# moddyz/stereo-to-multiview-cuda

Measured on AMD Instinct MI355X. Metric: stereo->8-view frames/sec @1080p d=64; cost-agg HBM GB/s vs roofline, higher is better.
Workload: dtype f32; 1 GPU; 1920x1080 synthetic stereo frame, D=64, zd=32, full stereo->8-view frame: cost init + cross aggregation + WTA + DCC/IRV x5/bilateral + 6 DIBR views + interlacing, one frame per GPU per step; stages=3, usd=34, lsd=17, views=8, aggregation=matrix pipe (stm_kernels_aggm.hip)

## Files before the change

include/stm_hip.h:

```cpp
#ifndef STM_HIP_H
#define STM_HIP_H

#ifdef __cplusplus
extern "C" {
#endif
#if defined(STM_BUILD) && defined(__GNUC__)
#pragma GCC visibility push(default)
#endif

int         stm_version(void);
void        stm_set_stream(void *hip_stream);
void       *stm_get_stream(void);
void        stm_set_error_mode(int mode);
const char *stm_last_error(void);
void        stm_release_workspace(void);
void        stm_prof_enable(int on);
void        stm_prof_reset(void);
int         stm_prof_read(const char *kernel, float *total_ms);
void        stm_set_agg_variant(int v);
int         stm_agg_path(int num_disp, int zero_disp, int num_rows, int num_cols, int usd, int stages);
int         stm_first_pass_path(int num_disp, int zero_disp, int num_rows, int num_cols, int usd, int stages);
void        stm_set_irv_paper_ratio(int on);
int         stm_set_irv_chunk(int entries);
int         stm_irv_path(int num_rows, int num_cols, int usd, int iterations, int device_flavour, int with_dcc);
int         stm_set_lens(int mode, double pitch, double slope, double centre);
int         stm_set_depth(int mode, float gain, float conv);
int         stm_set_depth_auto(float disp_lo, float disp_hi, float max_gain, int clip_permille, float rate, float *d_state);
int         stm_set_antialias(int mode, float strength, int max_radius, float gate);
void        stm_get_antialias(int out_mode[2], float out[2]);
int         stm_set_align(int mode, float a, float b, float c);
int         stm_set_align_auto(int radius, float rate, float *d_state);
void        stm_get_align(int out_mode[2], float out[4]);
int         stm_set_balance(int mode, const unsigned char *lut768);
int         stm_set_balance_auto(int max_shift, float rate, int *d_state);
void        stm_get_balance(int out_mode[2], float *out_rate, unsigned char out_lut[768]);
int         stm_set_cut(int mode, int thresh_permille, int min_gap, int *d_state);
void        stm_get_cut(int out[3]);
int         stm_set_layout(int layout, int tiles_x, int tiles_y, int order, int filter);
void        stm_get_layout(int *out);
int         stm_set_output(int format, int matrix, int pitch, int uv_row);
void        stm_get_output(int out[4]);
int         stm_set_overlay(int mode, const unsigned char *d_overlay, int ov_rows, int ov_cols, int x0, int y0, float disparity);
void        stm_get_overlay(int out[5], float *disparity);
void        stm_set_quilt_lds_limit(int bytes);
int         stm_set_packing(int packing, int swap, int filter, int gap);
void        stm_get_packing(int *out);
void        stm_set_ref_quirks(int on);

void stm_ci_adcensus(unsigned char *img_l, unsigned char *img_r, float **cost_l, float **cost_r,
                     float ad_coeff, float census_coeff, int num_disp, int zero_disp,
                     int num_rows, int num_cols, int elem_sz);
void stm_d_ci_adcensus(unsigned char *d_img_l, unsigned char *d_img_r,
                       float **d_adcensus_cost_l, float **d_adcensus_cost_r,
                       float **h_adcensus_cost_l, float **h_adcensus_cost_r,
                       float *d_adcensus_cost_memory,
                       float ad_coeff, float census_coeff, int num_disp, int zero_disp,
                       int num_rows, int num_cols, int elem_sz);

void stm_ca_cross(unsigned char *img, unsigned char **cross, float **cost, float **acost,
                  float ucd, float lcd, int usd, int lsd,
                  int num_disp, int num_rows, int num_cols, int elem_sz);
void stm_d_ca_cross(unsigned char *d_img, float **d_cost,
                    float **d_acost, float **h_acost, float *d_acost_memory,
                    unsigned char **d_cross,
                    float ucd, float lcd, int usd, int lsd,
                    int num_disp, int num_rows, int num_cols, int elem_sz);

void stm_dc_wta(float **cost, float *disp, int num_disp, int zero_disp, int num_rows, int num_cols);
void stm_d_dc_wta(float **d_cost, float *d_disp, int num_disp, int zero_disp, int num_rows, int num_cols);
void stm_dc_subpixel(float **cost, float *disp, int num_disp, int zero_disp, int num_rows, int num_cols);
void stm_d_dc_subpixel(float **d_cost, float *d_disp, int num_disp, int zero_disp, int num_rows, int num_cols);
void stm_dc_hslo(float **cost, float *disp, unsigned char *img_l, unsigned char *img_r,
                 float T, float H1, float H2, int num_disp, int zero_disp,
                 int num_rows, int num_cols, int elem_sz);
void stm_d_dc_hslo(float **d_cost, float *d_disp, unsigned char *d_img_l, unsigned char *d_img_r,
                   float T, float H1, float H2, int num_disp, int zero_disp,
                   int num_rows, int num_cols, int elem_sz);

void stm_dr_dcc(unsigned char *outliers_l, unsigned char *outliers_r, float *disp_l, float *disp_r,
                int num_rows, int num_cols);
void stm_d_dr_dcc(unsigned char *d_outliers_l, unsigned char *d_outliers_r, float *d_disp_l, float *d_disp_r,
                  int num_rows, int num_cols);
void stm_dr_irv(float *disp, unsigned char *outliers, unsigned char **cross, int thresh_s, float thresh_h,
                int num_rows, int num_cols, int num_disp, int zero_disp, int usd, int iterations);
void stm_d_dr_irv(float *d_disp, unsigned char *d_outliers, unsigned char **d_cross, int thresh_s, float thresh_h,
                  int num_rows, int num_cols, int num_disp, int zero_disp, int usd, int iterations);
void stm_dr_interp(float *disp, unsigned char *outliers, unsigned char *img, int num_rows, int num_cols, int elem_sz);
void stm_d_dr_interp(float *d_disp, unsigned char *d_outliers, unsigned char *d_img, int num_rows, int num_cols, int elem_sz);
void stm_filter_bilateral_1(float *img, int radius, float sigma_color, float sigma_spatial,
                            int num_rows, int num_cols, int num_disp);
void stm_d_filter_bilateral_1(float *d_img, int radius, float sigma_color, float sigma_spatial,
                              int num_rows, int num_cols, int num_disp);
void stm_filter_gaussian_1(float *img, int radius, float sigma_spatial, int num_rows, int num_cols);
void stm_d_filter_gaussian_1(float *d_img, int radius, float sigma_spatial, int num_rows, int num_cols);
void stm_filter_bleed_1(unsigned char *img, int radius, int num_rows, int num_cols);
void stm_d_filter_bleed_1(unsigned char *d_img, int radius, int num_rows, int num_cols);
void stm_filter_median(float *img, int num_rows, int num_cols);
void stm_d_filter_median(float *d_img, int num_rows, int num_cols);

void stm_dibr_occl(unsigned char *occl_l, unsigned char *occl_r, float *disp_l, float *disp_r,
                   int num_rows, int num_cols);
void stm_d_dibr_occl(unsigned char *d_occl_l, unsigned char *d_occl_r, float *d_disp_l, float *d_disp_r,
                     int num_rows, int num_cols);
void stm_dibr_occl_to_mask(float *mask_l, float *mask_r, unsigned char *occl_l, unsigned char *occl_r,
// ... 228 lines not shown
```

stereo-to-multiview-cuda_amd/_lib.py:

```python
import ctypes as C
import os

HERE = os.path.dirname(os.path.abspath(__file__))
LIB_PATH = os.path.join(HERE, "libstm_hip.so")
if os.environ.get("STM_LIB") == "timing":
    LIB_PATH = os.path.join(HERE, "libstm_hip_timing.so")

u8p = C.POINTER(C.c_uint8)
f32p = C.POINTER(C.c_float)
u32p = C.POINTER(C.c_uint32)
u8pp = C.POINTER(u8p)
f32pp = C.POINTER(f32p)
vp = C.c_void_p
i, f, d = C.c_int, C.c_float, C.c_double

PROTOS = {
    "stm_version": ([], i),
    "stm_set_stream": ([vp], None),
    "stm_get_stream": ([], vp),
    "stm_set_error_mode": ([i], None),
    "stm_last_error": ([], C.c_char_p),
    "stm_release_workspace": ([], None),
    "stm_prof_enable": ([i], None),
    "stm_prof_reset": ([], None),
    "stm_prof_read": ([C.c_char_p, f32p], i),
    "stm_set_agg_variant": ([i], None),
    "stm_agg_path": ([i, i, i, i, i, i], i),
    "stm_first_pass_path": ([i, i, i, i, i, i], i),
    "stm_set_irv_paper_ratio": ([i], None),
    "stm_set_irv_chunk": ([i], i),
    "stm_irv_path": ([i, i, i, i, i, i], i),
    "stm_set_ref_quirks": ([i], None),
    "stm_set_lens": ([i, d, d, d], i),
    "stm_set_layout": ([i, i, i, i, i], i),
    "stm_get_layout": ([C.POINTER(C.c_int)], None),
    "stm_set_output": ([i, i, i, i], i),
    "stm_get_output": ([C.POINTER(C.c_int)], None),
    "stm_set_overlay": ([i, vp, i, i, i, i, f], i),
    "stm_get_overlay": ([C.POINTER(C.c_int), f32p], None),
    "stm_set_quilt_lds_limit": ([i], None),
    "stm_set_packing": ([i, i, i, i], i),
    "stm_get_packing": ([C.POINTER(C.c_int)], None),
    "stm_set_depth": ([i, f, f], i),
    "stm_set_depth_auto": ([f, f, f, i, f, vp], i),
    "stm_set_antialias": ([i, f, i, f], i),
    "stm_get_antialias": ([C.POINTER(C.c_int), f32p], None),
    "stm_set_align": ([i, f, f, f], i),
    "stm_set_align_auto": ([i, f, vp], i),
    "stm_get_align": ([C.POINTER(C.c_int), f32p], None),
    "stm_set_balance": ([i, u8p], i),
    "stm_set_balance_auto": ([i, f, vp], i),
    "stm_get_balance": ([C.POINTER(C.c_int), f32p, u8p], None),
    "stm_set_cut": ([i, i, i, vp], i),
    "stm_get_cut": ([C.POINTER(C.c_int)], None),
    "stm_ci_adcensus": ([u8p, u8p, f32pp, f32pp, f, f, i, i, i, i, i], None),
    "stm_d_ci_adcensus": ([vp, vp, vp, vp, f32pp, f32pp, vp, f, f, i, i, i, i, i], None),
    "stm_ca_cross": ([u8p, u8pp, f32pp, f32pp, f, f, i, i, i, i, i, i], None),
    "stm_d_ca_cross": ([vp, vp, vp, f32pp, vp, vp, f, f, i, i, i, i, i, i], None),
    "stm_dc_wta": ([f32pp, f32p, i, i, i, i], None),
    "stm_d_dc_wta": ([vp, vp, i, i, i, i], None),
    "stm_dc_subpixel": ([f32pp, f32p, i, i, i, i], None),
    "stm_d_dc_subpixel": ([vp, vp, i, i, i, i], None),
    "stm_dc_hslo": ([f32pp, f32p, u8p, u8p, f, f, f, i, i, i, i, i], None),
    "stm_d_dc_hslo": ([vp, vp, vp, vp, f, f, f, i, i, i, i, i], None),
    "stm_dr_dcc": ([u8p, u8p, f32p, f32p, i, i], None),
    "stm_d_dr_dcc": ([vp, vp, vp, vp, i, i], None),
    "stm_dr_irv": ([f32p, u8p, u8pp, i, f, i, i, i, i, i, i], None),
    "stm_d_dr_irv": ([vp, vp, vp, i, f, i, i, i, i, i, i], None),
    "stm_dr_interp": ([f32p, u8p, u8p, i, i, i], None),
    "stm_d_dr_interp": ([vp, vp, vp, i, i, i], None),
    "stm_filter_bilateral_1": ([f32p, i, f, f, i, i, i], None),
    "stm_d_filter_bilateral_1": ([vp, i, f, f, i, i, i], None),
    "stm_filter_gaussian_1": ([f32p, i, f, i, i], None),
    "stm_d_filter_gaussian_1": ([vp, i, f, i, i], None),
    "stm_filter_bleed_1": ([u8p, i, i, i], None),
    "stm_d_filter_bleed_1": ([vp, i, i, i], None),
    "stm_filter_median": ([f32p, i, i], None),
    "stm_generate_gaussian_kernel": ([f32p, i, f], None),
    "stm_d_filter_median": ([vp, i, i], None),
    "stm_dibr_occl": ([u8p, u8p, f32p, f32p, i, i], None),
    "stm_d_dibr_occl": ([vp, vp, vp, vp, i, i], None),
    "stm_dibr_occl_to_mask": ([f32p, f32p, u8p, u8p, i, i], None),
    "stm_d_dibr_occl_to_mask": ([vp, vp, vp, vp, i, i], None),
    "stm_dibr_dbm": ([u8p, u8p, u8p, f32p, f32p, u8p, u8p, f32p, f32p, f, i, i, i], None),
    "stm_d_dibr_dbm": ([vp, vp, vp, vp, vp, vp, vp, vp, vp, f, i, i, i], None),
    "stm_dibr_dbm_lin": ([u8p, u8p, u8p, f32p, f32p, u8p, u8p, f32p, f32p, f, i, i, i], None),
    "stm_d_dibr_dbm_lin": ([vp, vp, vp, vp, vp, vp, vp, vp, vp, f, i, i, i], None),
    "stm_dibr_dfm": ([u8p, u8p, u8p, f32p, f32p, f, i, i, i], None),
    "stm_d_dibr_dfm": ([vp, vp, vp, vp, vp, f, i, i, i], None),
    "stm_mux_multiview": ([u8pp, u8p, i, f, i, i, i, i, i], None),
    "stm_d_mux_multiview": ([vp, vp, i, f, i, i, i, i, i], None),
    "stm_mux_multiview_lens": ([u8pp, u8p, i, i, d, d, d, i, i, i, i, i], None),
    "stm_d_mux_multiview_lens": ([vp, vp, i, i, d, d, d, i, i, i, i, i], None),
    "stm_quilt_multiview": ([u8pp, u8p, i, i, i, i, i, i, i, i, i, i], None),
    "stm_d_quilt_multiview": ([vp, vp, i, i, i, i, i, i, i, i, i, i], None),
    "stm_mux_overlay": ([u8p, u8p, i, i, i, i, f, i, f, i, d, d, d, i, i, i, i, i, i, i], None),
    "stm_d_mux_overlay": ([vp, vp, i, i, i, i, f, i, f, i, d, d, d, i, i, i, i, i, i, i], None),
    "stm_d_demux_sbs": ([vp, vp, vp, i, i, i, i], None),
    "stm_demux_nv12": ([u8p, u8p, u8p, i, u8p, i, i, i, i, i, i], None),
    "stm_d_demux_nv12": ([vp, vp, vp, i, vp, i, i, i, i, i, i], None),
    "stm_mux_nv12": ([u8p, i, u8p, i, u8p, i, i, i, i], None),
    "stm_d_mux_nv12": ([vp, i, vp, i, vp, i, i, i, i], None),
    "stm_demux_packed": ([u8p, u8p, u8p, i, i, i, i, i, i, i, i], None),
    "stm_d_demux_packed": ([vp, vp, vp, i, i, i, i, i, i, i, i], None),
    "stm_demux_nv12_packed": ([u8p, u8p, u8p, i, u8p, i, i, i, i, i, i, i, i, i, i], None),
    "stm_d_demux_nv12_packed": ([vp, vp, vp, i, vp, i, i, i, i, i, i, i, i, i, i], None),
    "stm_adcensus_stm": ([u8p, f32p, f32p, u8p, i, i, i, i, i, i, i, f, i, i, f, f, f, f, i, i, i, f], None),
    "stm_d_adcensus_stm": ([vp, vp, vp, vp, i, i, i, i, i, i, i, f, i, i, f, f, f, f, i, i, i, f, i], None),
    "stm_d_adcensus_stm_t": ([vp, vp, vp, vp, i, i, i, i, i, i, i, f, i, i, f, f, f, f, i, i, i, f, i, vp, vp, vp, f, i, f], None),
    "stm_d_adcensus_stm_nv12": ([vp, i, vp, i, i, vp, vp, vp, i, i, i, i, i, i, i, f, i, i, f, f, f, f, i, i, i, f, i, vp, vp, vp, vp, f, i, f,
                                 vp, vp], None),
# ... 82 lines not shown
```

stereo-to-multiview-cuda_amd/csrc/stm_api.hip:

```cpp
#include "stm_common.h"
#include <initializer_list>
#include <mutex>
#include "../../include/stm_hip.h"

#include <map>
#include <stdio.h>
#include <stdlib.h>
#include <string.h>
#include <tuple>
#include <vector>

using namespace stm;

namespace {

struct DevTable {
    float *d = nullptr;
    size_t n = 0;
};
std::map<std::tuple<int, int, float, float>, DevTable> g_tables;

int cur_dev()
{
    int dev = 0;
// ... 51 lines not shown
const float *bilateral_one_value_table(int D, int zd, float sigma_spatial, float sigma_color)
{
    if (D < 1 || D >= (1 << 19) || zd < 0 || zd >= 4096) return nullptr;
    return dev_table(3, D * 4096 + zd, sigma_spatial, sigma_color, (size_t)D, fill_bil1);
}

void sync() { STM_CHECK(hipStreamSynchronize(stream())); }

template <class T> T *up(const T *h, size_t n)
{
    T *d = Workspace::get<T>(n);
    STM_CHECK(hipMemcpyAsync(d, h, n * sizeof(T), hipMemcpyHostToDevice, stream()));
    return d;
}
template <class T> void down(T *h, const T *d, size_t n)
{
    STM_CHECK(hipMemcpyAsync(h, d, n * sizeof(T), hipMemcpyDeviceToHost, stream()));
}
float *up_planes(float **planes, int D, size_t HW)
{
    float *slab = Workspace::get<float>((size_t)D * HW);
    for (int d = 0; d < D; ++d)
        STM_CHECK(hipMemcpyAsync(slab + (size_t)d * HW, planes[d], HW * sizeof(float), hipMemcpyHostToDevice, stream()));
    return slab;
}
void down_planes(float **planes, const float *slab, int D, size_t HW)
{
    for (int d = 0; d < D; ++d)
        STM_CHECK(hipMemcpyAsync(planes[d], slab + (size_t)d * HW, HW * sizeof(float), hipMemcpyDeviceToHost, stream()));
}

struct Arms {
    u8 *up, *down, *left, *right;
};

struct Dim { const char *name; int v, lo; };
bool args_ok(const char *fn, std::initializer_list<Dim> dims)
{
    if (api_outermost()) clear_failed();
    for (const Dim &d : dims)
        if (d.v < d.lo) {
            char msg[160];
            snprintf(msg, sizeof msg, "%s: %s = %d, must be >= %d", fn, d.name, d.v, d.lo);
            fail(msg, d.name, __FILE__, __LINE__);
            return false;
        }
    return true;
}


void core_ci(const u8 *d_img_l, const u8 *d_img_r, Vol cl, Vol cr, uint32_t *pk_l, uint32_t *pk_r, float ad_coeff,
             float census_coeff, int D, int zd, int H, int W, int elem_sz, bool packed_ready = false,
             uint32_t **census_out = nullptr, uint32_t *const *census_ready = nullptr)
{
    size_t HW = (size_t)H * W;
    uint32_t *cen_l = census_ready ? census_ready[0] : Workspace::get<uint32_t>(HW), *cen_r = census_ready ? census_ready[1] : Workspace::get<uint32_t>(HW);
    if (!packed_ready) {
        launch_pack_bgrx(d_img_l, pk_l, H, W, elem_sz);
        launch_pack_bgrx(d_img_r, pk_r, H, W, elem_sz);
    }
    if (!census_ready) launch_census32_pair(pk_l, cen_l, pk_r, cen_r, H, W);
    if (census_out) {
        census_out[0] = cen_l;
        census_out[1] = cen_r;
        return;
    }
    const float *lut = rho_table(ad_coeff, census_coeff);
    launch_cost_init(pk_l, pk_r, cen_l, cen_r, cl, cr, lut, lut + 768, D, zd, H, W);
    if (ref_quirks()) launch_cost_quirks(pk_l, pk_r, cen_l, cen_r, cl, cr, lut, lut + 768, D, zd, H, W);
}

static bool agg_on_matrix_pipe(int usd, int H, int W) { return (agg_variant() / 10000) % 10 != 1 && aggm_supports(usd, H, W); }
static bool stages_hslo(int stages) { return (stages & 0x100) != 0; }
static bool stages_subpix(int stages) { return (stages & 0x200) != 0; }
int frame_agg_path(int D, int zd, int H, int W, int usd, int stages)
{
    if (D < 1 || H < 1 || W < 1 || !agg_on_matrix_pipe(usd, H, W)) return 0;
    return 1 | aggm_frame_path(D, zd, H, W, usd, stages_hslo(stages), stages_subpix(stages));
}
int frame_first_pass_path(int D, int zd, int H, int W, int usd, int stages)
{
    if (D < 1 || H < 1 || W < 1 || !agg_on_matrix_pipe(usd, H, W)) return 0;
    return aggm_frame_hc2_parts(D, zd, H, W, usd, stages_hslo(stages), stages_subpix(stages));
}
void core_agg(Vol cost, Vol scratch, const Arms &a, int D, int H, int W, int usd)
{
    if (agg_on_matrix_pipe(usd, H, W) && launch_aggm_stage(cost, cost, a.up, a.down, a.left, a.right, D, H, W, usd)) return;
    if (!scratch.base && !scratch.tab) scratch = vol_slab(Workspace::get<float>((size_t)D * H * W), (size_t)H * W);
    launch_agg_h(cost, scratch, a.left, a.right, D, H, W);
    launch_agg_v(scratch, cost, a.up, a.down, D, H, W, usd);
    launch_agg_v(cost, scratch, a.up, a.down, D, H, W, usd);
    launch_agg_h(scratch, cost, a.left, a.right, D, H, W);
}
Arms carve_arms(size_t HW)
{
    u8 *m = Workspace::get<u8>(4 * HW);
    return Arms{m, m + HW, m + 2 * HW, m + 3 * HW};
}
Arms arms_from_table(unsigned char **d_cross)
{
    u8 *h[4];
    STM_CHECK(hipMemcpyAsync(h, d_cross, sizeof h, hipMemcpyDeviceToHost, stream()));
    sync();
    return Arms{h[0], h[1], h[2], h[3]};
}

void core_bilateral(float *d_img, int radius, float sigma_color, float sigma_spatial, int H, int W, int D)
{
    size_t HW = (size_t)H * W;
    float *tmp = Workspace::get<float>(HW);
    launch_bilateral(d_img, tmp, gauss2d_table(radius, sigma_spatial), gauss1d_table(D, sigma_color), radius, H, W, D);
    STM_CHECK(hipMemcpyAsync(d_img, tmp, HW * sizeof(float), hipMemcpyDeviceToDevice, stream()));
}

void core_dbm(u8 *d_out, const u8 *d_l, const u8 *d_r, const float *disp_l, const float *disp_r, const float *mask_l,
              const float *mask_r, float shift, int H, int W, int elem_sz, int g_radius, float g_sigma, bool linear = false)
{
    size_t HW = (size_t)H * W;
    float *blend = Workspace::get<float>(HW);
    launch_gaussian_max(mask_r, blend, gauss2d_table(g_radius, g_sigma), g_radius, g_sigma, H, W, true);
    launch_view_synth(d_out, d_l, d_r, disp_l, disp_r, mask_l, mask_r, blend, shift, H, W, elem_sz, linear);
}

void dbm_device(const char *fn, unsigned char *d_img_out, unsigned char *d_img_in_l, unsigned char *d_img_in_r, float *d_disp_l,
                float *d_disp_r, float *d_mask_l, float *d_mask_r, float shift, int num_rows, int num_cols, int elem_sz, bool linear)
{
    if (!args_ok(fn, {{"num_rows", num_rows, 1}, {"num_cols", num_cols, 1}, {"elem_sz", elem_sz, 3}})) return;
    Workspace::begin((size_t)num_rows * num_cols * 4 + 1024);
    if (elem_sz > 3)
        STM_CHECK(hipMemsetAsync(d_img_out, 0, (size_t)num_rows * num_cols * elem_sz, stream()));
    core_dbm(d_img_out, d_img_in_l, d_img_in_r, d_disp_l, d_disp_r, d_mask_l, d_mask_r, shift, num_rows, num_cols, elem_sz,
             10, 15.0f, linear);
}
void dbm_host(const char *fn, unsigned char *img_out, unsigned char *img_in_l, unsigned char *img_in_r, float *disp_l, float *disp_r,
              float *mask_l, float *mask_r, float shift, int num_rows, int num_cols, int elem_sz, bool linear)
{
    if (!args_ok(fn, {{"num_rows", num_rows, 1}, {"num_cols", num_cols, 1}, {"elem_sz", elem_sz, 3}})) return;
    size_t HW = (size_t)num_rows * num_cols;
    Workspace::begin(3 * HW * elem_sz + 20 * HW + 8192);
    u8 *l = up(img_in_l, HW * elem_sz), *r = up(img_in_r, HW * elem_sz), *o = Workspace::get<u8>(HW * elem_sz);
    float *dl = up(disp_l, HW), *dr = up(disp_r, HW), *ml = up(mask_l, HW), *mr = up(mask_r, HW);
    STM_CHECK(hipMemsetAsync(o, 0, HW * elem_sz, stream()));
    core_dbm(o, l, r, dl, dr, ml, mr, shift, num_rows, num_cols, elem_sz, 7, 10.0f, linear);
    down(img_out, o, HW * elem_sz);
    sync();
}

bool mux_geom_ok(int N, float angle, int elem_sz, float *y_interval, float *inv_y_interval, int *ymod_out)
{
    float yi = mux_y_interval(N, angle, elem_sz);
    if (!(fabsf(yi) < 1.0e9f)) {
        fail("mux_multiview: y_interval is not finite (tan(angle) == 0 or angle is not a number)", "angle", __FILE__, __LINE__);
        return false;
    }
    int ymod = (int)roundf(yi);
    if (ymod == 0) {
        fail("mux_multiview: round(y_interval) == 0 (angle too steep)", "ymod", __FILE__, __LINE__);
        return false;
    }
    if (y_interval) *y_interval = yi;
    if (inv_y_interval) *inv_y_interval = 1.0f / yi;
    if (ymod_out) *ymod_out = ymod;
    return true;
}
void core_mux(const u8 *const *d_views, u8 *d_out, int N, float angle, int Hin, int Win, int Hout, int Wout, int elem_sz,
              int variant)
// ... 1690 lines not shown
    } else if (pack_on) {
        launch_demux_packed(img_l, img_r, pin, H, W, elem_sz);
        fused_split = false;
    } else if (nv && (agg_variant() / 100) % 10 != 6) {
        for (int i = 0; i < 6; ++i) pre[i] = Workspace::get<uint32_t>(HW);
        launch_front_nv12(img_l, img_r, pre[0], pre[1], pre[2], pre[3], pre[4], pre[5], nv->y, nv->pitch_y, nv->uv, nv->pitch_uv, H, W,
                          elem_sz, nv->matrix);
    } else if (nv) {
        launch_demux_nv12(img_l, img_r, nv->y, nv->pitch_y, nv->uv, nv->pitch_uv, H, W, elem_sz, nv->matrix);
        fused_split = false;
    } else if (fused_split && (agg_variant() / 100) % 10 != 6) {
        for (int i = 0; i < 6; ++i) pre[i] = Workspace::get<uint32_t>(HW);
        launch_front(img_l, img_r, pre[0], pre[1], pre[2], pre[3], pre[4], pre[5], d_img_sbs, H, num_cols_sbs, W, elem_sz);
    } else if (fused_split) {
        for (int i = 0; i < 4; ++i) pre[i] = Workspace::get<uint32_t>(HW);
        launch_demux_sbs_packed(img_l, img_r, pre[0], pre[1], pre[2], pre[3], d_img_sbs, H, num_cols_sbs, W, elem_sz);
    } else {
        launch_demux_sbs(img_l, img_r, d_img_sbs, H, num_cols_sbs, W, elem_sz);
    }
    Arms al, ar;
    const bool hslo = stages_hslo(stages), subpix = stages_subpix(stages);
    const bool interp = (stages & 0x400) != 0;
    const bool linwarp = (stages & 0x800) != 0;
    stages &= 0xff;
    frame_disparity(img_l, img_r, d_disp_l, d_disp_r, al, ar, H, W, elem_sz, num_disp, zero_disp, ad_coeff, census_coeff, ucd,
                    lcd, usd, lsd, thresh_s, thresh_h, stages >= 2, hslo, fused_split ? pre : nullptr, subpix, interp);
    if (hist) {
        float *c[2] = {d_disp_l, d_disp_r};
        const float *q[2] = {hist->disp_l, hist->disp_r};
        const bool split = split_hist || pack_on;
        const u8 *prev_l = hist->img_l, *prev_r = hist->img_r;
        if (pack_on && !nv) {
            u8 *ul = Workspace::get<u8>(IMG), *ur = Workspace::get<u8>(IMG);
            PackInput prev = pin;
            prev.frame = hist->sbs;
            launch_demux_packed(ul, ur, prev, H, W, elem_sz);
            prev_l = ul;
            prev_r = ur;
        }
        const u8 *im[2] = {split ? img_l : d_img_sbs, split ? img_r : d_img_sbs}, *ip[2] = {split ? prev_l : hist->sbs, split ? prev_r : hist->sbs};
        const size_t off[2] = {0, split ? 0 : (size_t)W * elem_sz};
        launch_disp_temporal(2, c, q, im, ip, off, H, W, split ? W : num_cols_sbs, elem_sz, hist->alpha, hist->thresh_color, hist->thresh_disp);
    }
    if (stages < 3) return;
    frame_render(img_l, img_r, d_disp_l, d_disp_r, d_interlaced, H, W, num_rows_out, num_cols_out, elem_sz, N, angle, linwarp);
    if (overlay().mode == 1) frame_overlay(d_interlaced, overlay(), lens(), layout(), N, angle, num_rows_out, num_cols_out, elem_sz);
}

bool frame_dims_ok(const char *fn, int num_rows, int num_cols_sbs, int num_cols, int num_rows_out, int num_cols_out, int elem_sz,
                   int num_views, int num_disp)
{
    return args_ok(fn, {{"num_rows", num_rows, 1}, {"num_cols_sbs", num_cols_sbs, 1}, {"num_cols", num_cols, 1},
                        {"num_rows_out", num_rows_out, 1}, {"num_cols_out", num_cols_out, 1}, {"elem_sz", elem_sz, 3},
                        {"num_views", num_views, 2}, {"num_disp", num_disp, 1}});
}

bool frame_packing_ok(const char *fn, int num_rows, int num_cols_sbs, int num_cols)
{
    const Packing pk = packing();
    return !pk.on() || packing_args_ok(fn, pk, num_rows, num_cols_sbs, num_cols, "num_cols", false, 0, 0, 0);
}
bool packing_unsupported(const char *fn)
{
    if (!packing().on()) return false;
    char msg[200];
    snprintf(msg, sizeof msg, "%s: a packing is set on this thread (stm_set_packing), which this call does not support: use d_adcensus_stm, "
             "d_adcensus_stm_t or d_adcensus_stm_nv12", fn);
    fail(msg, "packing", __FILE__, __LINE__);
    return true;
}

}

extern "C" {

int stm_agg_path(int num_disp, int zero_disp, int num_rows, int num_cols, int usd, int stages)
{
    return frame_agg_path(num_disp, zero_disp, num_rows, num_cols, usd, stages);
}
int stm_first_pass_path(int num_disp, int zero_disp, int num_rows, int num_cols, int usd, int stages)
{
    return frame_first_pass_path(num_disp, zero_disp, num_rows, num_cols, usd, stages);
}

void stm_d_adcensus_stm(unsigned char *d_img_sbs, float *d_disp_l, float *d_disp_r, unsigned char *d_interlaced,
                        int num_rows, int num_cols_sbs, int num_cols, int num_rows_out, int num_cols_out, int elem_sz,
                        int num_views, float angle, int num_disp, int zero_disp, float ad_coeff, float census_coeff,
                        float ucd, float lcd, int usd, int lsd, int thresh_s, float thresh_h, int stages)
{
    if (!frame_dims_ok("d_adcensus_stm", num_rows, num_cols_sbs, num_cols, num_rows_out, num_cols_out, elem_sz, num_views, num_disp)) return;
    if (!frame_packing_ok("d_adcensus_stm", num_rows, num_cols_sbs, num_cols)) return;
    if (stages & 0x2000) {
        fail("d_adcensus_stm: stages 0x2000 (temporal stabilisation) needs the history arguments of d_adcensus_stm_t", "stages", __FILE__,
             __LINE__);
        return;
    }
    frame_device("d_adcensus_stm", d_img_sbs, d_disp_l, d_disp_r, d_interlaced, num_rows, num_cols_sbs, num_cols, num_rows_out, num_cols_out,
                 elem_sz, num_views, angle, num_disp, zero_disp, ad_coeff, census_coeff, ucd, lcd, usd, lsd, thresh_s, thresh_h, stages, nullptr);
}

void stm_d_adcensus_stm_t(unsigned char *d_img_sbs, float *d_disp_l, float *d_disp_r, unsigned char *d_interlaced,
                          int num_rows, int num_cols_sbs, int num_cols, int num_rows_out, int num_cols_out, int elem_sz,
                          int num_views, float angle, int num_disp, int zero_disp, float ad_coeff, float census_coeff,
                          float ucd, float lcd, int usd, int lsd, int thresh_s, float thresh_h, int stages,
                          unsigned char *d_prev_img_sbs, float *d_prev_disp_l, float *d_prev_disp_r, float alpha, int thresh_color,
                          float thresh_disp)
{
    const char *fn = "d_adcensus_stm_t";
    if (!frame_dims_ok(fn, num_rows, num_cols_sbs, num_cols, num_rows_out, num_cols_out, elem_sz, num_views, num_disp)) return;
    if (!frame_packing_ok(fn, num_rows, num_cols_sbs, num_cols)) return;
    TemporalHist hist = {d_prev_img_sbs, d_prev_disp_l, d_prev_disp_r, alpha, thresh_color, thresh_disp};
    bool run = false;
    if (stages & 0x2000) {
        const int nset = (d_prev_img_sbs != nullptr) + (d_prev_disp_l != nullptr) + (d_prev_disp_r != nullptr);
        const size_t HW = (size_t)num_rows * num_cols;
        if (!temporal_params_ok(fn, alpha, thresh_color, thresh_disp)) return;
        if ((stages & 0xff) < 2) {
            fail("d_adcensus_stm_t: stages 0x2000 (temporal stabilisation) needs the refinement stages (2 or 3)", "stages", __FILE__, __LINE__);
            return;
        }
        if (nset != 0 && nset != 3) {
            fail("d_adcensus_stm_t: the three history pointers must be all null (first frame) or all set", "d_prev_img_sbs, d_prev_disp_l, d_prev_disp_r",
                 __FILE__, __LINE__);
            return;
        }
        if (nset == 3 && !packing().on() && num_cols_sbs < 2 * num_cols) {
            fail("d_adcensus_stm_t: stages 0x2000 (temporal stabilisation) needs num_cols_sbs >= 2 * num_cols", "num_cols_sbs", __FILE__, __LINE__);
            return;
        }
        if (nset == 3 && (maps_overlap(d_prev_disp_l, d_disp_l, HW) || maps_overlap(d_prev_disp_l, d_disp_r, HW) ||
                          maps_overlap(d_prev_disp_r, d_disp_l, HW) || maps_overlap(d_prev_disp_r, d_disp_r, HW))) {
            fail("d_adcensus_stm_t: a history map must not alias d_disp_l or d_disp_r", "d_prev_disp_l, d_prev_disp_r", __FILE__, __LINE__);
            return;
        }
        run = nset == 3;
    }
    frame_device(fn, d_img_sbs, d_disp_l, d_disp_r, d_interlaced, num_rows, num_cols_sbs, num_cols, num_rows_out, num_cols_out, elem_sz,
                 num_views, angle, num_disp, zero_disp, ad_coeff, census_coeff, ucd, lcd, usd, lsd, thresh_s, thresh_h, stages & ~0x2000,
                 run ? &hist : nullptr);
}

void stm_d_adcensus_stm_nv12(unsigned char *d_y, int pitch_y, unsigned char *d_uv, int pitch_uv, int matrix, float *d_disp_l, float *d_disp_r,
                             unsigned char *d_interlaced, int num_rows, int num_cols_sbs, int num_cols, int num_rows_out, int num_cols_out,
                             int elem_sz, int num_views, float angle, int num_disp, int zero_disp, float ad_coeff, float census_coeff,
                             float ucd, float lcd, int usd, int lsd, int thresh_s, float thresh_h, int stages,
                             unsigned char *d_prev_img_l, unsigned char *d_prev_img_r, float *d_prev_disp_l, float *d_prev_disp_r, float alpha,
                             int thresh_color, float thresh_disp, unsigned char *d_img_l, unsigned char *d_img_r)
{
    const char *fn = "d_adcensus_stm_nv12";
    if (!frame_dims_ok(fn, num_rows, num_cols_sbs, num_cols, num_rows_out, num_cols_out, elem_sz, num_views, num_disp)) return;
    if (packing().on()) {
        if (!packing_args_ok(fn, packing(), num_rows, num_cols_sbs, num_cols, "num_cols", true, pitch_y, pitch_uv, matrix)) return;
    } else if (!nv12_args_ok(fn, num_rows, num_cols_sbs, num_cols, "num_cols", pitch_y, pitch_uv, matrix)) return;
    if ((d_img_l != nullptr) != (d_img_r != nullptr)) {
        fail("d_adcensus_stm_nv12: d_img_l and d_img_r must be both null (the split images stay in the workspace) or both set", "d_img_l, d_img_r",
             __FILE__, __LINE__);
        return;
    }
    TemporalHist hist = {nullptr, d_prev_disp_l, d_prev_disp_r, alpha, thresh_color, thresh_disp, d_prev_img_l, d_prev_img_r};
    Nv12Input nv = {d_y, d_uv, pitch_y, pitch_uv, matrix, d_img_l, d_img_r};
    bool run = false;
    if (stages & 0x2000) {
        const int nset = (d_prev_img_l != nullptr) + (d_prev_img_r != nullptr) + (d_prev_disp_l != nullptr) + (d_prev_disp_r != nullptr);
        const size_t HW = (size_t)num_rows * num_cols, IMG = HW * elem_sz;
        if (!temporal_params_ok(fn, alpha, thresh_color, thresh_disp)) return;
        if ((stages & 0xff) < 2) {
// ... 505 lines not shown
```

stereo-to-multiview-cuda_amd/csrc/stm_common.h:

```cpp
#pragma once
#include <hip/hip_runtime.h>
#include <stddef.h>
#include <stdint.h>

typedef unsigned char u8;

namespace stm {

void fail(const char *what, const char *expr, const char *file, int line);
bool failed();
void clear_failed();
struct ApiNest { ApiNest(); ~ApiNest(); };
bool api_outermost();
void release_host_frame_bufs();
bool nv12_args_ok(const char *fn, int num_rows, int num_cols_sbs, int num_cols, const char *cols_name, int pitch_y, int pitch_uv, int matrix);
#define STM_CHECK(expr)                                                                  \
    do {                                                                                 \
        hipError_t _e = (expr);                                                          \
        if (_e != hipSuccess) ::stm::fail(hipGetErrorString(_e), #expr, __FILE__, __LINE__); \
    } while (0)
#define STM_CHECK_LAUNCH() STM_CHECK(hipGetLastError())
#define STM_LAUNCH(...)                                     \
    do {                                                    \
        if (!::stm::failed()) hipLaunchKernelGGL(__VA_ARGS__); \
// ... 244 lines not shown
void set_overlay(const Overlay &o);
bool overlay_params_ok(const char *fn, const void *ov, bool check_ptr, int ov_rows, int ov_cols, int x0, int y0, float disparity);
void frame_overlay(u8 *d_frame, const Overlay &ov, const Lens &ln, const Layout &lo, int num_views, float angle, int Hout, int Wout,
                   int elem_sz);
void launch_overlay(u8 *out, const u8 *ov, int ov_rows, int ov_cols, int x0, int y0, float disparity, int N, const Lens &ln,
                    float y_interval, float inv_y_interval, int ymod, const Layout &lo, int Hout, int Wout, int elem_sz);
struct Antialias {
    int mode;
    float strength;
    int max_radius;
    float gate;
};
Antialias antialias();
void set_antialias(const Antialias &a);
bool antialias_params_ok(const char *fn, float strength, int max_radius, float gate);
void launch_view_prefilter(int nimg, u8 *const *out, const u8 *const *in, const float *const *disp, int H, int W, int elem_sz, int num_views,
                           float strength, int max_radius, float gate, float gain, float conv, const float *state);
void launch_depth_fit(float *state, uint32_t *hist, const float *disp_l, const float *disp_r, int H, int W, float disp_lo, float disp_hi,
                      float max_gain, int clip_permille, float rate, bool fresh);
struct Align {
    int mode;
    float a, b, c;
    int radius;
    float rate;
    float *d_state;
};
Align align();
void set_align(const Align &a);
bool align_params_ok(const char *fn, int mode, float a, float b, float c);
bool align_auto_params_ok(const char *fn, int radius, float rate);
bool align_size_ok(const char *fn, int num_rows, int num_cols);
size_t align_profile_words(int H);
size_t align_sad_words(int radius);
void launch_align_measure(float *state, int *nvalid, uint32_t *prof, uint32_t *sad, const PackInput *in, const u8 *img_l, const u8 *img_r,
                          int H, int W, int elem_sz, int radius, float rate, bool fresh);
void launch_align_frame(u8 *out, const PackInput *in, const u8 *img, int H, int W, int elem_sz, float a, float b, float c, const float *state);
struct Balance {
    int mode;
    u8 lut[768];
    int max_shift;
    float rate;
    int *d_state;
};
Balance balance_default();
Balance balance();
void set_balance(const Balance &b);
bool balance_params_ok(const char *fn, int mode, const u8 *lut768);
bool balance_auto_params_ok(const char *fn, int max_shift, float rate);
bool balance_size_ok(const char *fn, int num_rows, int num_cols);
int balance_rate_q(float rate);
constexpr size_t BALANCE_HIST_WORDS = 1536, BALANCE_STATE_WORDS = 769;
void launch_balance_measure(int *state, uint32_t *hist, const PackInput *in, const u8 *img_l, const u8 *img_r, int H, int W, int elem_sz,
                            int max_shift, int rate_q, bool fresh);
void launch_balance_frame(u8 *out, const PackInput *in, const u8 *img, int H, int W, int elem_sz, const u8 *lut768, const int *state);
struct Cut {
    int mode;
    int thresh_permille, min_gap;
    int *d_state;
};
Cut cut_default();
Cut cut();
void set_cut(const Cut &c);
bool cut_params_ok(const char *fn, int thresh_permille, int min_gap);
bool cut_size_ok(const char *fn, int num_rows, int num_cols);
constexpr size_t CUT_SIG_WORDS = 256, CUT_STATE_WORDS = 260;
constexpr int CUT_DEFAULT_THRESH = 370;
void launch_cut_detect(int *state, uint32_t *sig, const PackInput *in, const u8 *img_l, int H, int W, int elem_sz, int thresh_permille,
                       int min_gap, void *reset0, void *reset1, void *reset2);
struct PQViews {
    const uint32_t *pk[2], *cen[2];
    float *a[2], *b[2];
    const u8 *armU[2], *armD[2], *armL[2], *armR[2];
    float *disp[2];
};
size_t pq_volume_floats(int D, int H, int W);
bool aggm_supports(int usd, int H, int W);
void launch_aggm_frame(const uint32_t *const *pk, const uint32_t *const *cen, const float *lut, float *const *vol_a, float *const *vol_b,
                       const u8 *const *armU, const u8 *const *armD, const u8 *const *armL, const u8 *const *armR, float *const *disp,
                       int D, int zd, int H, int W, int usd, bool keep_volume = false, uint32_t *htab_ready = nullptr, uint32_t *vtab_ready = nullptr,
                       bool v2_read_later = false);
size_t aggm_frame_htab_dwords(int D, int H, int W, int usd, bool keep_volume);
size_t aggm_frame_vtab_dwords(int D, int zd, int H, int W, int usd, bool keep_volume, bool v2_read_later, int *rec, int *top, bool *col);
bool aggm_frame_px(int D, int zd, int H, int W, int usd, bool keep_volume, bool v2_read_later);
int aggm_frame_path(int D, int zd, int H, int W, int usd, bool keep_volume, bool v2_read_later);
int aggm_frame_hc2_parts(int D, int zd, int H, int W, int usd, bool keep_volume, bool v2_read_later);
bool launch_aggm_stage(Vol in, Vol out, const u8 *armU, const u8 *armD, const u8 *armL, const u8 *armR, int D, int H, int W, int usd);
size_t aggm_stage_bytes(int D, int H, int W, int usd);
bool aggh_supports(int usd, int D);
size_t aggh_table_dwords(int nviews, int H, int W);
void launch_hwin_table(PQViews &v, int nviews, uint32_t *tab, int H, int W);
void launch_pq_hsr(PQViews &v, int nviews, const uint32_t *tab, int D, int zd, int H, int W, bool px = false);
bool aggv_supports(int usd);
int aggv_table_top();
int aggv_table_rec();
void launch_pq_v12q(PQViews &v, int nviews, const uint32_t *tab, int rec, int H, int W, int G, int NC);
void launch_pq_v12r(PQViews &v, int nviews, const uint32_t *tab, int H, int W, int G);
void launch_vcol_table(PQViews &v, int nviews, uint32_t *tab, int H, int W);
size_t aggv_col_table_dwords(int nviews, int H, int W);
void launch_to_pq(Vol in, float *pq, int D, int H, int W, uint32_t *odd = nullptr);
void launch_from_pq(const float *pq, Vol out, int D, int H, int W);
void launch_hslo_wta(int nviews, const Vol *cost, const u8 *const *img_a, const u8 *const *img_b, const int *osign,
                     float *const *disp, float T, float H1, float H2, int D, int zd, int H, int W, int elem_sz);
void launch_hslo_wta_pq(int nviews, float *const *cost_pq, float *const *acc_pq, const u8 *const *img_a, const u8 *const *img_b,
                        const int *osign, float *const *disp, float T, float H1, float H2, int D, int zd, int H, int W, int elem_sz);

void rho_luts(float ad_coeff, float census_coeff, float *lut_ad , float *lut_census );
void gaussian_kernel_2d(float *kernel, int radius, float sigma);
void gaussian_kernel_1d(float *kernel, int size, float sigma);
float mux_y_interval(int num_views, float angle, int elem_sz);

}
```

stereo-to-multiview-cuda_amd/csrc/stm_kernels_aggh.hip:

```cpp
#include "stm_hwin.h"
#include <cstdlib>

namespace stm {

__global__ __launch_bounds__(256) void stm_k_hwin_table(PQViews v, uint32_t *__restrict__ tab, int H, int W, int nTx)
{
    __shared__ uint32_t ev_all[4][4 * 96];
    const int wv = threadIdx.x >> 6, y = blockIdx.y, view = blockIdx.z;
    const int x0 = (blockIdx.x * 4 + wv) * 64, x = x0 + (threadIdx.x & 63);
    const u8 *__restrict__ armL = view ? v.armL[1] : v.armL[0], *__restrict__ armR = view ? v.armR[1] : v.armR[0];
    int aL = 0, aR = 0;
    if (x < W) {
        aL = armL[(size_t)y * W + x];
        aR = armR[(size_t)y * W + x];
    }
    hwin_build(tab + (size_t)view * H * nTx * HR_REC, ev_all[wv], y, x0, aL, aR, W, nTx);
}

template <int EXP, bool PX>
__global__ __launch_bounds__(64, 3) void stm_k_pq_hsr(PQViews pv, const uint32_t *__restrict__ htab, int D, int zd, int H, int W, int G, int NC, int nTx,
                                                      int parts, int nviews)
{
    const int part = blockIdx.x % parts, rest = blockIdx.x / parts, y = rest % H, view = rest / H;
    if (view >= nviews) return;
    const int per = (nTx + parts - 1) / parts, t0 = part * per, t1 = min(nTx, t0 + per);
    if (t0 >= t1) return;
    const int l = threadIdx.x;
    const float *in = view ? pv.a[1] : pv.a[0];
    float *disp_row = (view ? pv.disp[1] : pv.disp[0]) + (size_t)y * W;
    const uint32_t *hrec = htab + ((size_t)(view * H + y) * nTx + t0) * HR_REC;
    const uint32_t cstride = (uint32_t)H * (uint32_t)G * 256u;
    const uint32_t nrec = (uint32_t)NC * cstride;
    const int vload = PX ? 4 * l : (l >> 4) * (int)cstride + (l & 15) * 16;
    const int vn = l & 15;
    const int vst = (l & 15) == 0 ? (l >> 4) * 16 : 0x7ffffff0;
    float vbig[4];
#pragma unroll
    for (int b = 0; b < 4; ++b) vbig[b] = (16 * b + (l & 15)) >= D ? 3.402823466e+38f : 0.0f;
    const int yG = y * G, Gm1 = G - 1, W4 = W * 4;
    const float zdf = (float)zd;
    asm volatile(R"ASM(
        .set HR_EXP, %[exp]
        .set HR_PX, %[px]
        ; ---------------------------------------------------------------- macros
        ; one block of a sweep: four MFMAs on one pixel group (its four registers = four window steps), the A operand (lanes 16 a + m =
        ; step a, pixel m) shared through CBSZ / ABID.  p = block index, acur / anxt = the A registers of this / the next block
        .macro HR_BLOCK p, acur, anxt
        s_set_gpr_idx_idx s30
        v_mfma_f32_16x16x1_4b_f32 v[120:135], v[\acur], v0, v[120:135] cbsz:2 abid:0
        v_cndmask_b32_e64 v[\anxt], 0, 1.0, s[36+2*((\p)+1):37+2*((\p)+1)]
        v_mfma_f32_16x16x1_4b_f32 v[120:135], v[\acur], v1, v[120:135] cbsz:2 abid:1
        s_add_u32 s30, s30, 4
        s_cmp_eq_u32 s30, s29
        s_cselect_b32 s30, 0, s30
        v_mfma_f32_16x16x1_4b_f32 v[120:135], v[\acur], v2, v[120:135] cbsz:2 abid:2
        v_mfma_f32_16x16x1_4b_f32 v[120:135], v[\acur], v3, v[120:135] cbsz:2 abid:3
        .endm
        .macro HR_PAIR b
        HR_BLOCK 2*(\b), 136, 137
        HR_BLOCK 2*(\b)+1, 137, 136
        .endm
        ; in: s84 = q0 (first group of the sweep inside the range), s85 = n (1 .. 22), s26 = ring index of the range start.
        ; out: s90 = entry block 22 - n, s30 = ring index of the sweep's first group
        .macro HR_SWEEP_ISSUE
        s_sub_u32 s90, 22, s85
        s_lshl_b32 s31, s84, 2
        s_add_u32 s30, s26, s31
        s_sub_u32 s31, s30, s29
        s_cmp_ge_u32 s30, s29
        s_cselect_b32 s30, s31, s30
        .endm
        ; the header and the 24 mask pairs (block p reads pair p + 1 for its successor, the entry block's own comes through M0) of
        ; tile s31 (index relative to t0) start travelling
        .macro HR_NEXT_MASKS
        s_lshl_b32 s31, s31, 8
        s_add_u32 s88, %[hrec_lo], s31
        s_addc_u32 s89, %[hrec_hi], 0
        s_load_dwordx2 s[86:87], s[88:89], 0x0
        .if (HR_EXP & 8) == 0
        s_load_dwordx16 s[36:51], s[88:89], 0x20
        s_load_dwordx16 s[52:67], s[88:89], 0x60
        s_load_dwordx16 s[68:83], s[88:89], 0xa0
        .endif
        .endm
        .macro HR_SWEEP_RUN
        s_lshl_b32 m0, s90, 1
        s_nop 0
        s_movrels_b64 s[94:95], s[36:37]      ; the entry block's mask
        v_cndmask_b32_e64 v136, 0, 1.0, s[94:95]
        v_cndmask_b32_e64 v137, 0, 1.0, s[94:95]
        s_set_gpr_idx_on s30, 0x2
        s_mul_i32 s31, s90, 56
        s_getpc_b64 s[92:93]
HR_pc_%=_\@:
        s_add_u32 s31, s31, HR_blk0_%=_\@-HR_pc_%=_\@+12
        s_add_u32 s92, s92, s31
        s_addc_u32 s93, s93, 0
        v_mfma_f32_16x16x1_4b_f32 v[120:135], v136, v0, 0 cbsz:2 abid:0
        s_setpc_b64 s[92:93]
HR_blk0_%=_\@:
        HR_PAIR 0
        HR_PAIR 1
        HR_PAIR 2
        HR_PAIR 3
        HR_PAIR 4
        HR_PAIR 5
        HR_PAIR 6
        HR_PAIR 7
        HR_PAIR 8
        HR_PAIR 9
        HR_PAIR 10
HR_end_%=_\@:
        .if (HR_end_%=_\@-HR_blk0_%=_\@) != 22*56
        .error "sweep blocks are not 56 bytes each"
        .endif
        s_set_gpr_idx_off
        s_nop 15
        s_nop 3
        .endm
        .macro HR_ZERO_ACC
        v_mov_b32 v120, 0
// ... 78 lines not shown
        v_min_i32_dpp v[\d2], v[\d2], v[\d2] row_ror:4 row_mask:0xf bank_mask:0xf
        v_min_i32_dpp v[\d3], v[\d3], v[\d3] row_ror:4 row_mask:0xf bank_mask:0xf
        v_min_i32_dpp v[\d0], v[\d0], v[\d0] row_ror:2 row_mask:0xf bank_mask:0xf
        v_min_i32_dpp v[\d1], v[\d1], v[\d1] row_ror:2 row_mask:0xf bank_mask:0xf
        v_min_i32_dpp v[\d2], v[\d2], v[\d2] row_ror:2 row_mask:0xf bank_mask:0xf
        v_min_i32_dpp v[\d3], v[\d3], v[\d3] row_ror:2 row_mask:0xf bank_mask:0xf
        v_min_i32_dpp v[\d0], v[\d0], v[\d0] row_ror:1 row_mask:0xf bank_mask:0xf
        v_min_i32_dpp v[\d1], v[\d1], v[\d1] row_ror:1 row_mask:0xf bank_mask:0xf
        v_min_i32_dpp v[\d2], v[\d2], v[\d2] row_ror:1 row_mask:0xf bank_mask:0xf
        v_min_i32_dpp v[\d3], v[\d3], v[\d3] row_ror:1 row_mask:0xf bank_mask:0xf
        .endm

        ; one step of the walk: tile s24; lb = the landing registers this step empties and refills
        .macro HR_STEP lb
        ; the groups loaded two steps ago (4 t + 9 .. 4 t + 12) -> ring (the first tile's came with the prologue)
        s_cmp_eq_u32 s24, %[t0]
        s_cbranch_scc1 HR_nomove_%=_\@
        .if (HR_EXP & 2) == 0
        .if HR_PX
        s_waitcnt vmcnt(24)                   ; issued since: 4 stores, 16 loads, 4 stores
        .else
        s_waitcnt vmcnt(12)                   ; issued since: 4 stores, 4 loads, 4 stores
        .endif
        .endif
        s_add_u32 s96, s26, 72                ; group 4 t + 9 = range start + 18 groups
        s_sub_u32 s31, s96, s29
        s_cmp_ge_u32 s96, s29
        s_cselect_b32 s96, s31, s96
        s_set_gpr_idx_on s96, 0x8
        HR_PUT4 \lb
        HR_PUT4 \lb+4
        HR_PUT4 \lb+8
        HR_PUT4 \lb+12
        s_set_gpr_idx_off
HR_nomove_%=_\@:
        ; groups 4 t + 17 .. 4 t + 20 (the new groups of tile t + 2) -> the landing registers just emptied
        s_lshl_b32 s97, s24, 2
        s_add_i32 s97, s97, 17
        HR_LOAD_GROUP \lb, 0
        HR_LOAD_GROUP \lb, 1
        HR_LOAD_GROUP \lb, 2
        HR_LOAD_GROUP \lb, 3
        ; ------------------------------------------------------------ the sweep of tile t (header and masks left after the last sweep)
        s_waitcnt lgkmcnt(0)
        s_mov_b32 s84, s86
        s_min_u32 s85, s87, 22
        s_cmp_eq_u32 s85, 0
        s_cbranch_scc1 HR_zero_%=_\@
        .if (HR_EXP & 1) == 0
        HR_SWEEP_ISSUE
        HR_SWEEP_RUN
        s_branch HR_wta_%=_\@
        .endif
HR_zero_%=_\@:
        HR_ZERO_ACC
HR_wta_%=_\@:
        ; the next tile's header and masks travel during WTA and the next ring update (the last tile reads its own again)
        s_add_i32 s31, s24, 1
        s_sub_u32 s91, %[t1], 1
        s_min_i32 s31, s31, s91
        s_sub_i32 s31, s31, %[t0]
        HR_NEXT_MASKS
        .if (HR_EXP & 4) == 0
        ; ------------------------------------------------------------ WTA (d_dc_wta.cu:19-34)
        s_cmp_eq_u32 s27, 0
        s_cbranch_scc1 HR_nofix_%=_\@
        v_max_f32 v120, v120, %[vb0]
        v_max_f32 v121, v121, %[vb0]
        v_max_f32 v122, v122, %[vb0]
        v_max_f32 v123, v123, %[vb0]
        v_max_f32 v124, v124, %[vb1]
        v_max_f32 v125, v125, %[vb1]
        v_max_f32 v126, v126, %[vb1]
        v_max_f32 v127, v127, %[vb1]
        v_max_f32 v128, v128, %[vb2]
        v_max_f32 v129, v129, %[vb2]
        v_max_f32 v130, v130, %[vb2]
        v_max_f32 v131, v131, %[vb2]
        v_max_f32 v132, v132, %[vb3]
        v_max_f32 v133, v133, %[vb3]
        v_max_f32 v134, v134, %[vb3]
        v_max_f32 v135, v135, %[vb3]
HR_nofix_%=_\@:
        ; per lane: the lowest of its four chunks, the lower chunk on ties; v[138:141] = that hypothesis (d = 16 b + n)
        HR_WTA_CHUNK 1, 151
        HR_WTA_CHUNK 2, 152
        HR_WTA_CHUNK 3, 153
        ; over the 16 hypothesis lanes: lowest cost (bit patterns: costs are never negative), then the lowest d among its holders
        HR_ROWMIN4 142, 143, 144, 145, 120, 121, 122, 123
        v_cmp_eq_u32_e64 s[94:95], v142, v120
        v_cmp_eq_u32_e64 s[96:97], v143, v121
        v_cmp_eq_u32_e64 s[98:99], v144, v122
        v_cmp_eq_u32_e64 s[90:91], v145, v123
        v_cndmask_b32_e64 v146, v150, v138, s[94:95]
        v_cndmask_b32_e64 v147, v150, v139, s[96:97]
        v_cndmask_b32_e64 v148, v150, v140, s[98:99]
        v_cndmask_b32_e64 v149, v150, v141, s[90:91]
        HR_ROWMIN4 142, 143, 144, 145, 146, 147, 148, 149
        v_cvt_f32_i32 v142, v142
        v_cvt_f32_i32 v143, v143
        v_cvt_f32_i32 v144, v144
        v_cvt_f32_i32 v145, v145
        v_subrev_f32 v142, %[zdf], v142
        v_subrev_f32 v143, %[zdf], v143
        v_subrev_f32 v144, %[zdf], v144
        v_subrev_f32 v145, %[zdf], v145
        .endif
        ; lane n == 0 of a pixel quad stores pixels 16 t + 4 q + i; pixels past the row are out of range (the whole offset is in
        ; the vector register, so the range check sees it).  Always four stores: a step's loads are counted against them
        s_lshl_b32 s31, s24, 6
        v_add_u32 v146, s31, %[vst]
        s_nop 0
        buffer_store_dword v142, v146, s[20:23], 0 offen
        buffer_store_dword v143, v146, s[20:23], 0 offen offset:4
        buffer_store_dword v144, v146, s[20:23], 0 offen offset:8
        buffer_store_dword v145, v146, s[20:23], 0 offen offset:12
        ; next tile
        s_add_u32 s26, s26, 16
        s_sub_u32 s31, s26, s29
        s_cmp_ge_u32 s26, s29
        s_cselect_b32 s26, s31, s26
        s_add_i32 s24, s24, 1
        .endm

        ; ---------------------------------------------------------------- setup
        s_mov_b64 s[16:17], %[in]
        s_and_b32 s17, s17, 0xffff
        s_mov_b32 s18, %[nrec]
        s_mov_b32 s19, 0x20000
        s_mov_b64 s[20:21], %[disp]
        s_and_b32 s21, s21, 0xffff
        s_mov_b32 s22, 0
        s_mov_b32 s23, 0x20000
        s_mov_b32 s24, %[t0]
        s_mov_b32 s25, %[t1]
        s_mov_b32 s26, 0                      ; the ring starts at the first tile's range start: group 4 t0 - 9 + k in registers 4 k ..
        s_movk_i32 s29, 88
        s_mov_b32 s31, 0
        HR_NEXT_MASKS
        v_mov_b32 v150, 0x7fffffff
        v_add_u32 v151, 16, %[vn]
        v_add_u32 v152, 32, %[vn]
        v_add_u32 v153, 48, %[vn]
        v_or_b32 v146, %[vb0], %[vb1]
        v_or3_b32 v146, v146, %[vb2], %[vb3]
        v_cmp_ne_u32 vcc, 0, v146
        s_cmp_lg_u64 vcc, 0
        s_cselect_b32 s27, 1, 0               ; D < 64: some lanes hold hypotheses that must not win
        ; the first tile's 22 groups straight into the ring, the second tile's new groups into the odd step's landing registers
        s_lshl_b32 s97, %[t0], 2
        s_sub_i32 s97, s97, 9
        HR_LOAD_GROUP 0, 0
        HR_LOAD_GROUP 0, 1
        HR_LOAD_GROUP 0, 2
        HR_LOAD_GROUP 0, 3
        HR_LOAD_GROUP 0, 4
        HR_LOAD_GROUP 0, 5
        HR_LOAD_GROUP 0, 6
        HR_LOAD_GROUP 0, 7
        HR_LOAD_GROUP 0, 8
        HR_LOAD_GROUP 0, 9
        HR_LOAD_GROUP 0, 10
        HR_LOAD_GROUP 0, 11
        HR_LOAD_GROUP 0, 12
        HR_LOAD_GROUP 0, 13
        HR_LOAD_GROUP 0, 14
        HR_LOAD_GROUP 0, 15
        HR_LOAD_GROUP 0, 16
        HR_LOAD_GROUP 0, 17
        HR_LOAD_GROUP 0, 18
        HR_LOAD_GROUP 0, 19
        HR_LOAD_GROUP 0, 20
        HR_LOAD_GROUP 0, 21
        HR_LOAD_GROUP 104, 0
        HR_LOAD_GROUP 104, 1
        HR_LOAD_GROUP 104, 2
        HR_LOAD_GROUP 104, 3
        ; four stores into an empty buffer keep the steps' count of outstanding operations uniform (4 loads + 4 stores each)
        buffer_store_dword v142, v146, s[20:23], 0 offen
        buffer_store_dword v142, v146, s[20:23], 0 offen
        buffer_store_dword v142, v146, s[20:23], 0 offen
        buffer_store_dword v142, v146, s[20:23], 0 offen
        s_mov_b32 s22, %[W4]
        .if (HR_EXP & 2) == 0
        .if HR_PX
        s_waitcnt vmcnt(20)                   ; the ring is in (behind it: 16 loads, 4 stores)
        .else
        s_waitcnt vmcnt(8)                    ; the ring is in
        .endif
        .endif
HR_loop_%=:
        HR_STEP 88
        s_cmp_ge_i32 s24, s25
        s_cbranch_scc1 HR_done_%=
        HR_STEP 104
        s_cmp_lt_i32 s24, s25
        s_cbranch_scc1 HR_loop_%=
HR_done_%=:
        s_waitcnt vmcnt(0) lgkmcnt(0)         ; nothing may be in flight when the wave ends
        .purgem HR_BLOCK
        .purgem HR_PAIR
        .purgem HR_SWEEP_ISSUE
        .purgem HR_NEXT_MASKS
        .purgem HR_SWEEP_RUN
        .purgem HR_ZERO_ACC
        .purgem HR_PUT4
        .purgem HR_LOAD_GROUP
        .purgem HR_WTA_CHUNK
        .purgem HR_ROWMIN4
        .purgem HR_STEP
        )ASM"
                 :
                 : [exp] "n"(EXP), [px] "n"(PX ? 1 : 0), [in] "s"(in), [disp] "s"(disp_row), [hrec_lo] "s"((uint32_t)(uintptr_t)hrec), [hrec_hi] "s"((uint32_t)((uintptr_t)hrec >> 32)),
                   [yG] "s"(yG), [Gm1] "s"(Gm1), [nrec] "s"(nrec), [W4] "s"(W4), [t0] "s"(t0), [t1] "s"(t1), [zdf] "s"(zdf),
                   [vload] "v"(vload), [vn] "v"(vn), [vst] "v"(vst), [vb0] "v"(vbig[0]),
                   [vb1] "v"(vbig[1]), [vb2] "v"(vbig[2]), [vb3] "v"(vbig[3])
                 : "memory", "scc", "vcc",
                   "s16", "s17", "s18", "s19", "s20", "s21", "s22", "s23", "s24", "s25", "s26", "s27", "s29", "s30", "s31", "s36", "s37", "s38", "s39",
                   "s40", "s41", "s42", "s43", "s44", "s45", "s46", "s47", "s48", "s49", "s50", "s51", "s52", "s53", "s54", "s55", "s56", "s57", "s58", "s59",
                   "s60", "s61", "s62", "s63", "s64", "s65", "s66", "s67", "s68", "s69", "s70", "s71", "s72", "s73", "s74", "s75", "s76", "s77", "s78", "s79",
                   "s80", "s81", "s82", "s83", "s84", "s85", "s86", "s87", "s88", "s89", "s90", "s91", "s92", "s93", "s94", "s95", "s96", "s97", "s98", "s99",
                   "v0", "v1", "v2", "v3", "v4", "v5", "v6", "v7", "v8", "v9", "v10", "v11", "v12", "v13", "v14", "v15", "v16", "v17", "v18", "v19",
                   "v20", "v21", "v22", "v23", "v24", "v25", "v26", "v27", "v28", "v29", "v30", "v31", "v32", "v33", "v34", "v35", "v36", "v37", "v38", "v39",
                   "v40", "v41", "v42", "v43", "v44", "v45", "v46", "v47", "v48", "v49", "v50", "v51", "v52", "v53", "v54", "v55", "v56", "v57", "v58", "v59",
                   "v60", "v61", "v62", "v63", "v64", "v65", "v66", "v67", "v68", "v69", "v70", "v71", "v72", "v73", "v74", "v75", "v76", "v77", "v78", "v79",
                   "v80", "v81", "v82", "v83", "v84", "v85", "v86", "v87", "v88", "v89", "v90", "v91", "v92", "v93", "v94", "v95", "v96", "v97", "v98", "v99",
                   "v100", "v101", "v102", "v103", "v104", "v105", "v106", "v107", "v108", "v109", "v110", "v111", "v112", "v113", "v114", "v115", "v116",
                   "v117", "v118", "v119", "v120", "v121", "v122", "v123", "v124", "v125", "v126", "v127", "v128", "v129", "v130", "v131", "v132", "v133",
                   "v134", "v135", "v136", "v137", "v138", "v139", "v140", "v141", "v142", "v143", "v144", "v145", "v146", "v147", "v148", "v149", "v150",
                   "v151", "v152", "v153");
}

bool aggh_supports(int usd, int D) { return usd >= 1 && usd <= HR_TOP && D >= 1 && D <= 64; }

size_t aggh_table_dwords(int nviews, int H, int W) { return (size_t)nviews * H * cdiv(W, 16) * HR_REC + 64; }

void launch_hwin_table(PQViews &v, int nviews, uint32_t *tab, int H, int W)
{
    const int nTx = cdiv(W, 16);
    STM_LAUNCH(stm_k_hwin_table, dim3(cdiv(nTx, 16), H, nviews), dim3(256), 0, stream(), v, tab, H, W, nTx);
    STM_CHECK_LAUNCH();
}

void launch_pq_hsr(PQViews &v, int nviews, const uint32_t *tab, int D, int zd, int H, int W, bool px)
{
    const int G = (W + 3) / 4, NC = (D + 15) / 16, nTx = cdiv(W, 16);
    int parts = (nTx + 5) / 10;
    parts = parts < 1 ? 1 : parts;
    const dim3 grid(nviews * H * parts);
#define STM_HSR_LAUNCH(E, GRID)                                                                                                       \
    {                                                                                                                                 \
        if (px) STM_LAUNCH((stm_k_pq_hsr<E, true>), GRID, dim3(64), 0, stream(), v, tab, D, zd, H, W, G, NC, nTx, parts, nviews);      \
        else STM_LAUNCH((stm_k_pq_hsr<E, false>), GRID, dim3(64), 0, stream(), v, tab, D, zd, H, W, G, NC, nTx, parts, nviews);        \
    }
#ifdef STM_TIMING
    if (const char *e = getenv("STM_HSR_PARTS")) parts = atoi(e);
    const dim3 gridt(nviews * H * parts);
    switch (timing_knobs()) {
    case 1: STM_HSR_LAUNCH(1, gridt); break;
    case 2: STM_HSR_LAUNCH(2, gridt); break;
    case 3: STM_HSR_LAUNCH(3, gridt); break;
    case 4: STM_HSR_LAUNCH(4, gridt); break;
    case 5: STM_HSR_LAUNCH(5, gridt); break;
    case 6: STM_HSR_LAUNCH(6, gridt); break;
    case 7: STM_HSR_LAUNCH(7, gridt); break;
    case 8: STM_HSR_LAUNCH(8, gridt); break;
    default: STM_HSR_LAUNCH(0, gridt); break;
    }
#else
    STM_HSR_LAUNCH(0, grid);
#endif
#undef STM_HSR_LAUNCH
    STM_CHECK_LAUNCH();
}

}
```

stereo-to-multiview-cuda_amd/csrc/stm_kernels_aggm.hip:

```cpp
#include "stm_hwin.h"

namespace stm {

typedef float f4 __attribute__((ext_vector_type(4)));

#define STM_MFMA16(m, b, acc, abid) __builtin_amdgcn_mfma_f32_16x16x1f32(m, b, acc, 2, abid, 0)
typedef float f16v __attribute__((ext_vector_type(16)));
typedef uint32_t u4v __attribute__((ext_vector_type(4)));
#define STM_MASKF(m) (__builtin_amdgcn_inverse_ballot_w64(m) ? 1.0f : 0.0f)
#define STM_BLOAD(rsrc, voff) __builtin_bit_cast(f4, __builtin_amdgcn_raw_buffer_load_b128(rsrc, voff, 0, 2))


template <int N> __device__ __forceinline__ float row_ror_f(float v)
{
    return __builtin_bit_cast(float, __builtin_amdgcn_update_dpp(0, __builtin_bit_cast(int, v), 0x120 + N, 0xf, 0xf, false));
}
template <int N> __device__ __forceinline__ int row_ror_i(int v) { return __builtin_amdgcn_update_dpp(0, v, 0x120 + N, 0xf, 0xf, false); }
__device__ __forceinline__ int wave_min_i(int v)
{
    v = min(v, row_ror_i<8>(v)); v = min(v, row_ror_i<4>(v)); v = min(v, row_ror_i<2>(v)); v = min(v, row_ror_i<1>(v));
    return min(min(__builtin_amdgcn_readlane(v, 0), __builtin_amdgcn_readlane(v, 16)),
               min(__builtin_amdgcn_readlane(v, 32), __builtin_amdgcn_readlane(v, 48)));
}
__device__ __forceinline__ int wave_max_i(int v)
// ... 370 lines not shown
                }
                int it = 1;
                for (; it + 2 <= n_it; it += 2) {
                    STM_HS_NEXT(ca)
                    STM_HS_MFMA(cb)
                    STM_HS_NEXT(cb)
                    STM_HS_MFMA(ca)
                }
                if (it < n_it) STM_HS_MFMA(cb)
#undef STM_HS_NEXT
#undef STM_HS_MFMA
            } else {
#pragma unroll
                for (int i = 0; i < 16; ++i) acc[i] = 0.f;
            }
            if (!WTA) {
#pragma unroll
                for (int cl = 0; cl < 4; ++cl) {
                    const f4 o = {acc[4 * cl], acc[4 * cl + 1], acc[4 * cl + 2], acc[4 * cl + 3]};
                    STM_BSTORE(rout[cl], (X0 >> 2) * 256 + l * 16, o);
                }
            } else {
                float bc[4];
                int bd[4];
#pragma unroll
                for (int i = 0; i < 4; ++i) { bc[i] = 3.402823466e+38f; bd[i] = 0; }
#pragma unroll
                for (int cl = 0; cl < 4; ++cl) {
                    const int d = (c0 + cl) * 16 + dd;
                    if (d < D) {
#pragma unroll
                        for (int i = 0; i < 4; ++i)
                            if (bc[i] > acc[4 * cl + i]) { bc[i] = acc[4 * cl + i]; bd[i] = d; }
                    }
                }
                const __amdgpu_buffer_rsrc_t rs = __builtin_amdgcn_make_buffer_rsrc((void *)(disp + row), 0, (uint32_t)W * 4u, 0x00020000);
#pragma unroll
                for (int i = 0; i < 4; ++i) {
                    const int bi = __builtin_bit_cast(int, bc[i]);
                    int m = bi;
                    m = min(m, row_ror_i<8>(m));
                    m = min(m, row_ror_i<4>(m));
                    m = min(m, row_ror_i<2>(m));
                    m = min(m, row_ror_i<1>(m));
                    int cand = (bi == m) ? bd[i] : 0x7fffffff;
                    cand = min(cand, row_ror_i<8>(cand));
                    cand = min(cand, row_ror_i<4>(cand));
                    cand = min(cand, row_ror_i<2>(cand));
                    cand = min(cand, row_ror_i<1>(cand));
                    if (ncs > 1) {
                        uint2 *slot = wb + (X0 - seg0 * TX + 4 * lb + i);
                        if (dd == 0) {
                            if (cs > 0) {
                                const uint2 pv = *slot;
                                if (!(m < (int)pv.x)) { m = (int)pv.x; cand = (int)pv.y; }
                            }
                            if (cs + 1 < ncs) *slot = make_uint2((uint32_t)m, (uint32_t)cand);
                        }
                        if (cs + 1 < ncs) continue;
                    }
                    __builtin_amdgcn_raw_buffer_store_b32(__builtin_bit_cast(uint32_t, (float)cand - (float)zd), rs,
                                                          dd == 0 ? (X0 + 4 * lb + i) * 4 : (int)0x7ffffff0, 0, 0);
                }
            }
        }
        __syncthreads();
        if (more) {
            int sl = slot0 + w;
            if (sl >= NJ) sl -= NJ;
#pragma unroll
            for (int k = 0; k < KP; ++k) tile[(k * NJ + sl) * 64 + l] = st[k];
            STM_HS_SN(sq + 1)
            slot0 += NW;
            if (slot0 >= NJ) slot0 -= NJ;
        }
        __syncthreads();
    }
  }
#undef STM_HS_LOAD
#undef STM_HS_ARMS
#undef STM_HS_SN
}

template <int NW, bool PX>
__global__ __launch_bounds__(64 * NW, (2 * NW) / 4) void stm_k_pq_hc(PQViews v, int D, int zd, int H, int W, int G, int NC, int HG, int nseg,
                                                                     int spl, const float *__restrict__ lut_g, int pad, int dbg)
{
    constexpr int NT = 64 * NW, TX = 16 * NW, NEWPX = 16 * NW;
    extern __shared__ f4 lds4[];
    const int NG = 4 * NW + 2 * HG, NJ = NG >> 2;
    f4 *tile = lds4;
    uint32_t *sn = (uint32_t *)(tile + 4 * NG * 16);
    int2 *sg = (int2 *)(sn + TX);
    const int SO = NEWPX + 2 * pad;
    uint2 *s_own = (uint2 *)(sg + NW), *s_oth = s_own + 2 * NEWPX;
    float *s_lut_ad = (float *)(s_oth + 2 * SO), *s_lut_c = s_lut_ad + 768;
    const int tid = threadIdx.x, l = tid & 63, w = __builtin_amdgcn_readfirstlane(tid >> 6);
    const int lb = l >> 4, dd = l & 15;
    const int part = blockIdx.x % spl, rest = blockIdx.x / spl, y = rest % H, view = rest / H;
    const int seg_per = (nseg + spl - 1) / spl, seg0 = part * seg_per, seg1 = min(nseg, seg0 + seg_per);
    if (seg0 >= seg1) return;
    f4 *__restrict__ out = (f4 *)(view ? v.b[1] : v.b[0]);
    const u8 *__restrict__ armL = view ? v.armL[1] : v.armL[0], *__restrict__ armR = view ? v.armR[1] : v.armR[0];
    const uint32_t *__restrict__ pk_own = view ? v.pk[1] : v.pk[0], *__restrict__ pk_oth = view ? v.pk[0] : v.pk[1];
    const uint32_t *__restrict__ cen_own = view ? v.cen[1] : v.cen[0], *__restrict__ cen_oth = view ? v.cen[0] : v.cen[1];
    const int sgn = view ? -1 : 1;
    const size_t row = (size_t)y * W;
    const uint32_t rowbytes = (uint32_t)G * 256u;
    for (int i = tid; i < 768 + 65; i += NT) s_lut_ad[i] = lut_g[i];
    uint2 so = make_uint2(0, 0), sx = make_uint2(0, 0);
    int aLn = 0, aRn = 0;
    f4 cst[4];
  const int ncs = (NC + 3) >> 2;
  for (int cs = 0; cs < ncs; ++cs) {
    const int c0 = 4 * cs;
    __amdgpu_buffer_rsrc_t rout[4];
#pragma unroll
    for (int cl = 0; cl < 4; ++cl)
        rout[cl] = __builtin_amdgcn_make_buffer_rsrc((void *)(out + ((size_t)min(c0 + cl, NC - 1) * H + y) * G * 16), 0, c0 + cl < NC ? rowbytes : 0u, 0x00020000);
    const __amdgpu_buffer_rsrc_t rpx = __builtin_amdgcn_make_buffer_rsrc((void *)(out + (size_t)y * G * 64), 0, PX ? 4u * rowbytes : 0u, 0x00020000);
#define STM_HC_FETCH(A0)                                                                           \
    {                                                                                              \
        const int x0_ = 4 * ((A0) - HG);                                                           \
        if (tid < NEWPX) {                                                                         \
            const int gx = min(max(x0_ + tid, 0), W - 1);                                          \
            so = make_uint2(pk_own[row + gx], cen_own[row + gx]);                                  \
        }                                                                                          \
        if (tid < SO) {                                                                            \
            const int gx = min(max(x0_ - pad + tid, 0), W - 1);                                    \
            sx = make_uint2(pk_oth[row + gx], cen_oth[row + gx]);                                  \
        }                                                                                          \
    }
#define STM_HC_STAGE(B)                                            \
    {                                                              \
        if (tid < NEWPX) s_own[(B) * NEWPX + tid] = so;            \
        if (tid < SO) s_oth[(B) * SO + tid] = sx;                  \
    }
#define STM_HC_COSTS(B, A0)                                                                                               \
    {                                                                                                                     \
        const int gi = 4 * w + lb, x0g = 4 * ((A0) - HG + gi);                                                            \
        const uint2 *own = s_own + (B) * NEWPX + gi * 4;                                                                  \
        const uint2 o0 = own[0], o1 = own[1], o2 = own[2], o3 = own[3];                                                   \
        const bool in0 = x0g >= 0 && x0g < W, in1 = x0g + 1 >= 0 && x0g + 1 < W, in2 = x0g + 2 >= 0 && x0g + 2 < W,       \
                   in3 = x0g + 3 >= 0 && x0g + 3 < W;                                                                     \
         \
         \
        _Pragma("unroll") for (int cl = 0; cl < 4; ++cl) {                                                                \
            f4 val = {0.f, 0.f, 0.f, 0.f};                                                                                \
            if (c0 + cl < NC) {                                                                              \
                const int d = (c0 + cl) * 16 + dd;                   \
                const uint2 *oth = s_oth + (B) * SO + gi * 4 + sgn * (d - zd) + pad;                                      \
                const uint2 q0 = oth[0], q1 = oth[1], q2 = oth[2], q3 = oth[3];                                           \
                const float a0 = s_lut_ad[__builtin_amdgcn_sad_u8(o0.x, q0.x, 0u)], c0 = s_lut_c[hamdist_q1(o0.y, q0.y)]; \
                const float a1 = s_lut_ad[__builtin_amdgcn_sad_u8(o1.x, q1.x, 0u)], c1 = s_lut_c[hamdist_q1(o1.y, q1.y)]; \
                const float a2 = s_lut_ad[__builtin_amdgcn_sad_u8(o2.x, q2.x, 0u)], c2 = s_lut_c[hamdist_q1(o2.y, q2.y)]; \
                const float a3 = s_lut_ad[__builtin_amdgcn_sad_u8(o3.x, q3.x, 0u)], c3 = s_lut_c[hamdist_q1(o3.y, q3.y)]; \
                const bool dok = d < D;                                                                                   \
                val.x = (in0 && dok) ? a0 + c0 : 0.f;                                                                     \
                val.y = (in1 && dok) ? a1 + c1 : 0.f;                                                                     \
                val.z = (in2 && dok) ? a2 + c2 : 0.f;                                                                     \
                val.w = (in3 && dok) ? a3 + c3 : 0.f;                                                                     \
            }                                                                                                             \
            cst[cl] = val;                                                                                                \
        }                                                                                                                 \
    }
#define STM_HC_ARMS(S)                                                          \
    if (tid < TX) {                                                             \
// ... 21 lines not shown
        __syncthreads();
        if (r0 + w < NJ) {
            STM_HC_COSTS(0, a0)
#pragma unroll
            for (int k = 0; k < 4; ++k) tile[(k * NJ + (NW * seg0 + r0 + w) % NJ) * 64 + l] = cst[k];
        }
    }
    __syncthreads();
    {
        const int a1 = 4 * NW * (seg0 + 1) + NG - 4 * NW;
        STM_HC_FETCH(a1)
        STM_HC_STAGE((seg0 + 1) & 1)
        STM_HC_ARMS(seg0)
        STM_HC_SN(seg0)
    }
    __syncthreads();
    int slot0 = (NW * seg0) % NJ;
    for (int sq = seg0; sq < seg1; ++sq) {
        const int X0 = sq * TX + 16 * w;
        const bool more = sq + 1 < seg1;
        if (more) {
            STM_HC_FETCH(4 * NW * (sq + 2) + NG - 4 * NW)
            STM_HC_ARMS(sq + 1)
        }
        if (X0 < W) {
            const uint32_t e = sn[16 * w + dd];
            const int srel = (int)(e & 0xffffu), nn = (int)(e >> 16);
            const int2 sgw = sg[w];
            const int G0r = __builtin_amdgcn_readfirstlane(sgw.x);
            const int n_it = STM_DBG(dbg, 1) ? 0 : __builtin_amdgcn_readfirstlane(sgw.y);
            f16v acc;
            if (n_it > 0) {
                int gs = 4 * slot0 + G0r;
                if (gs >= NG) gs -= NG;
                const f4 *p = tile + (lb * NG + gs) * 16 + dd;
                int t = 4 * G0r + lb - srel;
#define STM_HS_NEXT(C)                                        \
    {                                                         \
        C = *p;                                               \
        p += 16;                                              \
        if (++gs == NG) { gs = 0; p -= NG * 16; }  \
    }
#define STM_HS_MFMA(C)                                                          \
    {                                                                           \
        const float m = ((unsigned)t < (unsigned)nn) ? 1.0f : 0.0f;             \
        t += 4;                                                                 \
        acc = STM_MFMA16(m, C.x, acc, 0);                                       \
        acc = STM_MFMA16(m, C.y, acc, 1);                                       \
        acc = STM_MFMA16(m, C.z, acc, 2);                                       \
        acc = STM_MFMA16(m, C.w, acc, 3);                                       \
    }
                f4 ca, cb;
                STM_HS_NEXT(ca)
                STM_HS_NEXT(cb)
                {
                    const float m = ((unsigned)t < (unsigned)nn) ? 1.0f : 0.0f;
                    t += 4;
                    const f16v z = {0.f, 0.f, 0.f, 0.f, 0.f, 0.f, 0.f, 0.f, 0.f, 0.f, 0.f, 0.f, 0.f, 0.f, 0.f, 0.f};
                    acc = STM_MFMA16(m, ca.x, z, 0);
                    acc = STM_MFMA16(m, ca.y, acc, 1);
                    acc = STM_MFMA16(m, ca.z, acc, 2);
                    acc = STM_MFMA16(m, ca.w, acc, 3);
                }
                int it = 1;
                for (; it + 2 <= n_it; it += 2) {
                    STM_HS_NEXT(ca)
                    STM_HS_MFMA(cb)
                    STM_HS_NEXT(cb)
                    STM_HS_MFMA(ca)
                }
                if (it < n_it) STM_HS_MFMA(cb)
#undef STM_HS_NEXT
#undef STM_HS_MFMA
            } else {
#pragma unroll
                for (int i = 0; i < 16; ++i) acc[i] = 0.f;
            }
            if (!PX) {
#pragma unroll
                for (int cl = 0; cl < 4; ++cl) {
                    const f4 o = {acc[4 * cl], acc[4 * cl + 1], acc[4 * cl + 2], acc[4 * cl + 3]};
                    if (!STM_DBG(dbg, 4)) STM_BSTORE(rout[cl], (X0 >> 2) * 256 + l * 16, o);
                }
            } else {
#pragma unroll
                for (int k = 0; k < 16; ++k)
                    if (!STM_DBG(dbg, 4))
                        __builtin_amdgcn_raw_buffer_store_b32(__builtin_bit_cast(uint32_t, (float)acc[k]), rpx,
                                                              (X0 + 4 * lb + (k & 3)) * 256 + (16 * (k >> 2) + dd) * 4, 0, 2);
            }
        }
        if (more) STM_HC_COSTS((sq + 1) & 1, 4 * NW * (sq + 1) + NG - 4 * NW)
        __syncthreads();
        if (more) {
            int sl = slot0 + w;
            if (sl >= NJ) sl -= NJ;
#pragma unroll
            for (int k = 0; k < 4; ++k) tile[(k * NJ + sl) * 64 + l] = cst[k];
            STM_HC_STAGE(sq & 1)
            STM_HC_SN(sq + 1)
            slot0 += NW;
            if (slot0 >= NJ) slot0 -= NJ;
        }
        __syncthreads();
    }
  }
#undef STM_HC_FETCH
#undef STM_HC_STAGE
#undef STM_HC_COSTS
#undef STM_HC_ARMS
#undef STM_HC_SN
}

constexpr int HC2_TX = 96, HC2_SR = HC2_TX + 64, HC2_HALO = 40, HC2_RING = 256, HC2_FRONT = HC2_TX + HC2_HALO;
typedef const float __attribute__((address_space(3))) *hc2_lds_cf;
constexpr size_t HC2_SMEM =(size_t)(HC2_RING + 3) * 256 + 2 * HC2_TX * 4 + 12 * 8 + (size_t)(2 * HC2_TX + 2 * HC2_SR) * 8 + (768 + 72) * 4;
__global__ __launch_bounds__(768, 6) void stm_k_pq_hc2(PQViews v, int D, int zd, int H, int W, int G, int nseg, int spl,
                                                       const float *__restrict__ lut_g, int dbg)
{
    constexpr int NW = 12, NT = 64 * NW, TX = HC2_TX, SR = HC2_SR;
    extern __shared__ f4 lds4[];
    float *ring = (float *)lds4;
    uint32_t *sn = (uint32_t *)(ring + (HC2_RING + 3) * 64);
    int2 *sg = (int2 *)(sn + 2 * TX);
    uint2 *s_l = (uint2 *)(sg + NW), *s_r = s_l + 2 * TX;
    float *s_lut_ad = (float *)(s_r + 2 * SR), *s_lut_c = s_lut_ad + 768;
    const int tid = threadIdx.x, l = tid & 63, w = __builtin_amdgcn_readfirstlane(tid >> 6);
    const int lb = l >> 4, dd = l & 15;
    const int part = blockIdx.x % spl, y = blockIdx.x / spl;
    const int seg_per = (nseg + spl - 1) / spl, seg0 = part * seg_per, seg1 = min(nseg, seg0 + seg_per);
    if (seg0 >= seg1) return;
    const int view = w >= NW / 2, wt = view ? w - NW / 2 : w;
    f4 *__restrict__ out = (f4 *)(view ? v.b[1] : v.b[0]);
    const uint32_t *__restrict__ pk_l = v.pk[0], *__restrict__ pk_r = v.pk[1], *__restrict__ cen_l = v.cen[0], *__restrict__ cen_r = v.cen[1];
    const int aview = tid >= TX, apx = aview ? tid - TX : tid;
    const u8 *__restrict__ armL = aview ? v.armL[1] : v.armL[0], *__restrict__ armR = aview ? v.armR[1] : v.armR[0];
    const size_t row = (size_t)y * W;
    const uint32_t rowbytes = (uint32_t)G * 256u;
    for (int i = tid; i < 768 + 65; i += NT) s_lut_ad[i] = lut_g[i];
    uint2 sl = make_uint2(0, 0), sr = make_uint2(0, 0);
    int aLn = 0, aRn = 0;
    float cst[8];
    const __amdgpu_buffer_rsrc_t rpx = __builtin_amdgcn_make_buffer_rsrc((void *)(out + (size_t)y * G * 64), 0, 4u * rowbytes, 0x00020000);
#define STM_HC2_FETCH(P0)                                                                          \
    {                                                                                              \
        if (tid < TX) {                                                                            \
            const int gx = min(max((P0) + tid, 0), W - 1);                                         \
            sl = make_uint2(pk_l[row + gx], cen_l[row + gx]);                                      \
        }                                                                                          \
        if (tid < SR) {                                                                            \
            const int gx = min(max((P0) - zd + tid, 0), W - 1);                                    \
            sr = make_uint2(pk_r[row + gx], cen_r[row + gx]);                                      \
        }                                                                                          \
    }
#define STM_HC2_STAGE(B)                                           \
    {                                                              \
        if (tid < TX) s_l[(B) * TX + tid] = sl;                    \
        if (tid < SR) s_r[(B) * SR + tid] = sr;                    \
    }
#define STM_HC2_COSTS(B)                                                                                                  \
    {                                                                                                                     \
        const uint2 *lp = s_l + (B) * TX + 8 * w, *rp = s_r + (B) * SR + 8 * w + l;                                       \
        _Pragma("unroll") for (int k = 0; k < 8; ++k) {                                                                   \
            const uint2 o = lp[k], q = rp[k];                                                                             \
            const float a = s_lut_ad[__builtin_amdgcn_sad_u8(o.x, q.x, 0u)], c = s_lut_c[hamdist_q1(o.y, q.y)];           \
            cst[k] = l < D ? a + c : 0.f;                                                                                 \
        }                                                                                                                 \
    }
#define STM_HC2_WRITE(P0)                                                              \
    _Pragma("unroll") for (int k = 0; k < 8; ++k) {                                    \
        const int rp_ = ((P0) + 8 * w + k) & (HC2_RING - 1);              \
        ring[rp_ * 64 + l] = cst[k];                                                   \
        if (rp_ < 3) ring[(HC2_RING + rp_) * 64 + l] = cst[k];                         \
    }
#define STM_HC2_ARMS(S)                                                         \
    if (tid < 2 * TX) {                                                         \
        const int x = min((S) * TX + apx, W - 1);                               \
        aLn = armL[row + x];                                                    \
        aRn = armR[row + x];                                                    \
    }
#define STM_HC2_SN(S)                                                                                                      \
    if (tid < 2 * TX) {                                                                                                    \
        const int x = (S) * TX + apx, org = (S) * TX - HC2_HALO;                                                           \
         \
        const int srel_ = x < W ? x - aLn - org : x - org, nn_ = x < W ? aLn + aRn : 0;                                    \
        sn[tid] = (uint32_t)srel_ | ((uint32_t)nn_ << 16);                                                                 \
                           \
        int lo_ = nn_ ? (srel_ >> 2) : 0x7fffffff, hi_ = nn_ ? ((srel_ + nn_ + 3) >> 2) : -0x7fffffff;                     \
        lo_ = min(lo_, row_ror_i<8>(lo_)); lo_ = min(lo_, row_ror_i<4>(lo_)); lo_ = min(lo_, row_ror_i<2>(lo_)); lo_ = min(lo_, row_ror_i<1>(lo_)); \
        hi_ = max(hi_, row_ror_i<8>(hi_)); hi_ = max(hi_, row_ror_i<4>(hi_)); hi_ = max(hi_, row_ror_i<2>(hi_)); hi_ = max(hi_, row_ror_i<1>(hi_)); \
        if ((tid & 15) == 0) sg[tid >> 4] = make_int2(lo_, hi_ - lo_);                                                     \
    }
    const int front0 = TX * seg0 + HC2_FRONT + zd;
    for (int r0 = 0; r0 < HC2_RING; r0 += TX) {
        const int p0 = front0 - HC2_RING + r0;
        STM_HC2_FETCH(p0)
        __syncthreads();
        STM_HC2_STAGE(0)
        __syncthreads();
        if (r0 + 8 * w < HC2_RING) {
            STM_HC2_COSTS(0)
            STM_HC2_WRITE(p0)
        }
    }
    __syncthreads();
    {
        STM_HC2_FETCH(front0)
        STM_HC2_STAGE((seg0 + 1) & 1)
        STM_HC2_ARMS(seg0)
        STM_HC2_SN(seg0)
    }
    __syncthreads();
    const int shear = view ? min(l, D - 1) - zd : 0;
    for (int sq = seg0; sq < seg1; ++sq) {
        const int X0 = sq * TX + 16 * wt;
        const int front = TX * sq + HC2_FRONT + zd;
        const bool more = sq + 1 < seg1;
        if (more) {
            STM_HC2_FETCH(front + TX)
            STM_HC2_ARMS(sq + 1)
        }
        if (X0 < W) {
            const uint32_t e = sn[16 * w + dd];
            const int srel = (int)(e & 0xffffu), nn = (int)(e >> 16);
            const int2 sgw = sg[w];
            const int G0r = __builtin_amdgcn_readfirstlane(sgw.x);
            const int n_it = STM_DBG(dbg, 1) ? 0 : __builtin_amdgcn_readfirstlane(sgw.y);
            f16v acc;
            if (n_it > 0) {
                uint32_t a = ((((unsigned)(sq * TX - HC2_HALO + 4 * G0r - shear) << 8) + 4u * l) & 0xffffu);
                int t = 4 * G0r + lb - srel;
#define STM_HS_NEXT(C)                                                        \
    {                                                                         \
        const hc2_lds_cf r_ = (hc2_lds_cf)(size_t)a;                          \
        C.x = r_[0]; C.y = r_[64]; C.z = r_[128]; C.w = r_[192];              \
        asm("v_add_u16_e32 %0, 0x400, %1" : "=v"(a) : "v"(a));                \
    }
#define STM_HS_MFMA(C)                                                          \
    {                                                                           \
        const float m = ((unsigned)t < (unsigned)nn) ? 1.0f : 0.0f;             \
        t += 4;                                                                 \
        acc = STM_MFMA16(m, C.x, acc, 0);                                       \
        acc = STM_MFMA16(m, C.y, acc, 1);                                       \
        acc = STM_MFMA16(m, C.z, acc, 2);                                       \
        acc = STM_MFMA16(m, C.w, acc, 3);                                       \
    }
                f4 ca, cb;
                STM_HS_NEXT(ca)
                STM_HS_NEXT(cb)
                {
                    const float m = ((unsigned)t < (unsigned)nn) ? 1.0f : 0.0f;
                    t += 4;
                    const f16v z = {0.f, 0.f, 0.f, 0.f, 0.f, 0.f, 0.f, 0.f, 0.f, 0.f, 0.f, 0.f, 0.f, 0.f, 0.f, 0.f};
                    acc = STM_MFMA16(m, ca.x, z, 0);
                    acc = STM_MFMA16(m, ca.y, acc, 1);
                    acc = STM_MFMA16(m, ca.z, acc, 2);
                    acc = STM_MFMA16(m, ca.w, acc, 3);
                }
                int it = 1;
                for (; it + 2 <= n_it; it += 2) {
                    STM_HS_NEXT(ca)
                    STM_HS_MFMA(cb)
                    STM_HS_NEXT(cb)
                    STM_HS_MFMA(ca)
                }
                if (it < n_it) STM_HS_MFMA(cb)
#undef STM_HS_NEXT
#undef STM_HS_MFMA
            } else {
#pragma unroll
                for (int i = 0; i < 16; ++i) acc[i] = 0.f;
            }
#pragma unroll
            for (int k = 0; k < 16; ++k)
                if (!STM_DBG(dbg, 4))
                    __builtin_amdgcn_raw_buffer_store_b32(__builtin_bit_cast(uint32_t, (float)acc[k]), rpx,
                                                          (X0 + 4 * lb + (k & 3)) * 256 + (16 * (k >> 2) + dd) * 4, 0, 2);
        }
        if (more) STM_HC2_COSTS((sq + 1) & 1)
        __syncthreads();
        if (more) {
            STM_HC2_WRITE(front)
            STM_HC2_STAGE(sq & 1)
            STM_HC2_SN(sq + 1)
        }
        __syncthreads();
    }
#undef STM_HC2_FETCH
#undef STM_HC2_STAGE
#undef STM_HC2_COSTS
#undef STM_HC2_WRITE
#undef STM_HC2_ARMS
#undef STM_HC2_SN
}

constexpr int VT_EV = 2 * 255 + 32;
__global__ __launch_bounds__(256) void stm_k_vwin_table(PQViews v, uint32_t *__restrict__ tab, int rec, int H, int W, int G, int nT, int top)
{
    __shared__ unsigned long long ev_all[4][VT_EV];
    const int l = threadIdx.x & 63, wv = threadIdx.x >> 6, g = blockIdx.x * 4 + wv, u = blockIdx.y, view = blockIdx.z;
    if (g >= G) return;
    unsigned long long *ev = ev_all[wv];
    const u8 *__restrict__ armU = view ? v.armU[1] : v.armU[0], *__restrict__ armD = view ? v.armD[1] : v.armD[0];
    const int b = l >> 4, i = l & 15, y = u * 16 + i, x = 4 * g + b;
    int s0 = 0, nn = 0;
    if (y < H && x < W) {
        const int aU = armU[(size_t)y * W + x], aD = armD[(size_t)y * W + x];
        s0 = y - aU;
        nn = aU + aD;
    }
    vwin_build(tab + ((size_t)(view * nT + u) * G + g) * rec, ev, u, top, s0, nn);
}

typedef __attribute__((address_space(4))) const uint32_t ctab32;
typedef __attribute__((address_space(4))) const unsigned long long ctab64;
struct V12Quad { f4 c; unsigned long long m0, m1, m2, m3; };
struct V12Sweep {
    const f4 *p;
    ctab64 *mk;
    int qs, n_it;
    V12Quad A;
};
#define STM_V12_LOAD(S, Q, RQ)                                                      \
    {                                                                               \
        Q.c = *S.p;                                                                 \
        Q.m0 = S.mk[0]; Q.m1 = S.mk[1]; Q.m2 = S.mk[2]; Q.m3 = S.mk[3];             \
        S.p += 64; S.mk += 4;                                                       \
        if (++S.qs == RQ) { S.qs = 0; S.p -= RQ * 64; }                \
        asm volatile("" ::: "memory"); __builtin_amdgcn_sched_barrier(0);           \
    }
#define STM_V12_ARRIVED(Q) __builtin_amdgcn_sched_barrier(0); asm volatile("" : : "v"(Q.c), "s"(Q.m0), "s"(Q.m1), "s"(Q.m2), "s"(Q.m3) : "memory");
#define STM_V12_MFMA(Q)                                                                                            \
    {                                                                                                              \
        float a0 = STM_MASKF(Q.m0), a1 = STM_MASKF(Q.m1), a2 = STM_MASKF(Q.m2), a3 = STM_MASKF(Q.m3);              \
        asm volatile("" : "+v"(a0), "+v"(a1), "+v"(a2), "+v"(a3));  \
        acc = __builtin_amdgcn_mfma_f32_16x16x1f32(a0, Q.c.x, acc, 0, 0, 0);                                       \
        acc = __builtin_amdgcn_mfma_f32_16x16x1f32(a1, Q.c.y, acc, 0, 0, 0);                                       \
        acc = __builtin_amdgcn_mfma_f32_16x16x1f32(a2, Q.c.z, acc, 0, 0, 0);                                       \
        acc = __builtin_amdgcn_mfma_f32_16x16x1f32(a3, Q.c.w, acc, 0, 0, 0);                                       \
    }
__device__ __forceinline__ void v12t_begin(V12Sweep &S, const f4 *ring_l, int RQ, int slot0, int u4, ctab32 *r, int K0, int n_it)
{
    int qs = slot0 + ((K0 >> 2) - u4);
    if (qs < 0) qs += RQ;
    if (qs >= RQ) qs -= RQ;
    S.qs = qs;
    S.n_it = n_it;
    S.p = ring_l + qs * 64;
    S.mk = (ctab64 *)(r + 8);
    STM_V12_LOAD(S, S.A, RQ)
}
#define STM_V12_MFMA0(Q)                                                                                           \
    {                                                                                                              \
        float a0 = STM_MASKF(Q.m0), a1 = STM_MASKF(Q.m1), a2 = STM_MASKF(Q.m2), a3 = STM_MASKF(Q.m3);              \
        asm volatile("" : "+v"(a0), "+v"(a1), "+v"(a2), "+v"(a3));                                                 \
        const f16v z = {0.f, 0.f, 0.f, 0.f, 0.f, 0.f, 0.f, 0.f, 0.f, 0.f, 0.f, 0.f, 0.f, 0.f, 0.f, 0.f};           \
        acc = __builtin_amdgcn_mfma_f32_16x16x1f32(a0, Q.c.x, z, 0, 0, 0);                                         \
        acc = __builtin_amdgcn_mfma_f32_16x16x1f32(a1, Q.c.y, acc, 0, 0, 0);                                       \
        acc = __builtin_amdgcn_mfma_f32_16x16x1f32(a2, Q.c.z, acc, 0, 0, 0);                                       \
        acc = __builtin_amdgcn_mfma_f32_16x16x1f32(a3, Q.c.w, acc, 0, 0, 0);                                       \
// ... 144 lines not shown
                const int ro = 16 * u * rsb;
#pragma unroll
                for (int i = 0; i < 4; ++i) {
                    const f4 o = {acc[i], acc[4 + i], acc[8 + i], acc[12 + i]};
                    if (!STM_DBG(dbg, 4)) __builtin_amdgcn_raw_buffer_store_b128(__builtin_bit_cast(u4v, o), rout, vo[i] + ro, 0, 2);
                }
                s2 += TQ;
                if (s2 >= RQ2) s2 -= RQ2;
            }
            __syncthreads();
            u += NTP;
            v12t_begin(S, ring2 + l, RQ2, s2, 4 * max(u, 0), trow + (size_t)min(max(u, 0), nT - 1) * tstep, K0n, n_itn);
        }
    }
#undef STM_V12_HDR
}

size_t pq_volume_floats(int D, int H, int W) { return (size_t)((D + 15) / 16) * H * ((W + 3) / 4) * 64; }

static size_t v12t_smem(int usd)
{
    const int TS = 48, UQ = (usd + 3) & ~3, LAG = (UQ + TS - 1) / TS + 1;
    return (size_t)(TS + 2 * UQ + TS * (LAG + 1) + UQ) * 256;
}
bool aggm_supports(int usd, int H, int W)
{
    if (usd > 255) usd = 255;
    return usd >= 1 && v12t_smem(usd) <= 160 * 1024 && (unsigned long long)H * ((W + 3) / 4) * 256ull < (1ull << 31);
}

template <bool QUAD> __global__ __launch_bounds__(256) void stm_k_from_pq(const f4 *__restrict__ in, Vol out, int D, int H, int W, int G)
{
    const int t = blockIdx.x * 256 + threadIdx.x, y = blockIdx.y, c = blockIdx.z;
    const int g = t >> 2, q = 4 * c + (t & 3);
    if (g >= G || 4 * q >= D) return;
    const f4 *src = in + (((size_t)c * H + y) * G + g) * 16 + 4 * (t & 3);
    const f4 d0 = src[0], d1 = src[1], d2 = src[2], d3 = src[3];
#pragma unroll
    for (int k = 0; k < 4; ++k) {
        const int x = 4 * g + k;
        if (x < W) store_quad<QUAD, false>(out, q, D, (size_t)y * W + x, make_float4(d0[k], d1[k], d2[k], d3[k]));
    }
}
void launch_from_pq(const float *pq, Vol out, int D, int H, int W)
{
    const int G = (W + 3) / 4, NC = (D + 15) / 16;
    if (out.quad) STM_LAUNCH(stm_k_from_pq<true>, dim3(cdiv(4 * G, 256), H, NC), dim3(256), 0, stream(), (const f4 *)pq, out, D, H, W, G);
    else STM_LAUNCH(stm_k_from_pq<false>, dim3(cdiv(4 * G, 256), H, NC), dim3(256), 0, stream(), (const f4 *)pq, out, D, H, W, G);
    STM_CHECK_LAUNCH();
}

static int hc_waves(int D, int zd, int usd)
{
    constexpr int NW = 8, NWC = 12;
    const int NC = (D + 15) / 16;
    const int HG = ((usd + 3) / 4 + 2) & ~1, NG = 4 * NW + 2 * HG, NGc = 4 * NWC + 2 * HG;
    int pad = zd > D - 1 - zd ? zd : D - 1 - zd;
    pad = (pad < 0 ? 0 : pad) + 15;
    const size_t smem_hc = (size_t)4 * NGc * 256 + 16 * NWC * 4 + 8 * NWC + (size_t)(2 * 16 * NWC + 2 * (16 * NWC + 2 * pad)) * 8 + (768 + 72) * 4;
    const size_t smem_hc8 = (size_t)4 * NG * 256 + 16 * NW * 4 + 8 * NW + (size_t)(2 * 16 * NW + 2 * (16 * NW + 2 * pad)) * 8 + (768 + 72) * 4;
    const bool hc_ok = (agg_variant() / 1000000) % 10 != 1 && (agg_variant() / 1000) % 10 == 0 && (NC <= 4 || (agg_variant() / 10) % 10 != 2);
    if (hc_ok && smem_hc <= 80 * 1024 && 16 * NWC + 2 * pad <= 64 * NWC) return NWC;
    if (hc_ok && smem_hc8 <= 80 * 1024 && 16 * NW + 2 * pad <= 64 * NW) return NW;
    return 0;
}

static int row_split(int nseg) { return nseg > 24 ? cdiv(nseg, 16) : 1; }
static bool chain_vregs(int usd) { return aggv_supports(usd) && (agg_variant() / 10000000) % 10 != 1; }
static bool chain_hregs(bool wta, int usd, int D) { return wta && aggh_supports(usd, D) && (agg_variant() / 100000000) % 10 != 1; }

static bool chain_px(bool from_costs, bool wta, int D, int zd, int usd)
{
    if (usd > 255) usd = 255;
    const int NC = (D + 15) / 16;
    return from_costs && NC == 4 && chain_vregs(usd) && (agg_variant() / 10000000) % 10 == 0 && chain_hregs(wta, usd, D) &&
           hc_waves(D, zd, usd) != 0;
}
bool aggm_frame_px(int D, int zd, int H, int W, int usd, bool keep_volume, bool v2_read_later)
{
    (void)H;
    (void)W;
    return !v2_read_later && chain_px(true, !keep_volume, D, zd, usd);
}

constexpr int HC2_SLOTS = 2 * 256;
static int hc2_parts(bool px, int D, int zd, int H, int W, int usd)
{
    const int HG = ((usd + 3) / 4 + 2) & ~1;
    if (!px || (agg_variant() / 1000000) % 10 == 2 || hc_waves(D, zd, usd) != 12) return 0;
    if (zd < 0 || zd >= D || D > 64 || 4 * HG > HC2_HALO) return 0;
    if (cdiv(W, HC2_TX) < 8 || H >= 8 * HC2_SLOTS) return 1;
    return 2 * row_split(cdiv(W, 2 * HC2_TX));
}

struct ChainPlan {
    bool regs, hregs;
    int hcw;
    int hc_nseg, hc_spl;
    int hc2_spl;
};
static ChainPlan chain_plan(bool from_costs, bool wta, int D, int zd, int H, int W, int usd, bool px)
{
    ChainPlan c;
    c.regs = chain_vregs(usd);
    c.hregs = chain_hregs(wta, usd, D);
    const bool fuse_cost = from_costs && (agg_variant() / 1000000) % 10 != 1;
    c.hcw = fuse_cost ? hc_waves(D, zd, usd) : 0;
    c.hc_nseg = c.hcw ? cdiv(W, 16 * c.hcw) : 0;
    c.hc_spl = row_split(c.hc_nseg);
    c.hc2_spl = fuse_cost && c.hcw ? hc2_parts(px, D, zd, H, W, usd) : 0;
    return c;
}
int aggm_frame_path(int D, int zd, int H, int W, int usd, bool keep_volume, bool v2_read_later)
{
    if (usd > 255) usd = 255;
    const ChainPlan c = chain_plan(true, !keep_volume, D, zd, H, W, usd, false);
    return (aggm_frame_px(D, zd, H, W, usd, keep_volume, v2_read_later) ? 2 : 0) | (c.regs ? 4 : 0) | (c.hregs ? 8 : 0) | (c.hcw << 8) |
           (c.hc_spl > 1 ? 1 << 16 : 0);
}

int aggm_frame_hc2_parts(int D, int zd, int H, int W, int usd, bool keep_volume, bool v2_read_later)
{
    if (usd > 255) usd = 255;
    return chain_plan(true, !keep_volume, D, zd, H, W, usd, aggm_frame_px(D, zd, H, W, usd, keep_volume, v2_read_later)).hc2_spl;
}

static void aggm_chain(PQViews &v, int nviews, bool from_costs, bool wta, const float *lut, int D, int zd, int H, int W, int usd,
                       uint32_t *htab_ready = nullptr, uint32_t *vtab_ready = nullptr, bool px = false)
{
    const int G = (W + 3) / 4, NC = (D + 15) / 16;
    if (usd > 255) usd = 255;
    constexpr int NW = 8;
    const int HG = ((usd + 3) / 4 + 2) & ~1, NG = 4 * NW + 2 * HG;
    const int nseg = cdiv(W, 16 * NW), nblk = ((nseg * H * nviews + 7) / 8) * 8;
    const size_t smem_h = (size_t)4 * NG * 256 + 16 * NW * 4;
    const int dbgh = timing_knobs();
    int pad = zd > D - 1 - zd ? zd : D - 1 - zd;
    pad = (pad < 0 ? 0 : pad) + 15;
    const size_t smem_cost = smem_h + (size_t)(4 * NG * 4 + 4 * pad + 768 + 72) * 4;
    const bool fuse_cost = from_costs && (agg_variant() / 1000000) % 10 != 1;
    const int spl = row_split(nseg);
    const ChainPlan plan = chain_plan(from_costs, wta, D, zd, H, W, usd, px && nviews == 2);
    const bool streaming = NG / 4 >= NW && (agg_variant() / 10) % 10 != 1 && (NC <= 4 || (agg_variant() / 10) % 10 != 2);
    constexpr int NTP = 3, TS = 16 * NTP;
    const int UQ = (usd + 3) & ~3, nT = (H + 15) / 16;
    const bool regs = plan.regs;
    const int rec = regs ? aggv_table_rec() : 8 + 8 * ((2 * usd + 21) / 4 + 2);
    const int LAG = (UQ + TS - 1) / TS + 1;
    const int RQ1 = (TS + 2 * UQ) / 4, RQ2 = (TS * (LAG + 1) + UQ) / 4;
    uint32_t *vtab = regs && vtab_ready ? vtab_ready : Workspace::get<uint32_t>(px ? aggv_col_table_dwords(nviews, H, W) : (size_t)nviews * nT * G * rec);
    const bool hregs = plan.hregs;
    uint32_t *htab = !hregs ? nullptr : htab_ready ? htab_ready : Workspace::get<uint32_t>(aggh_table_dwords(nviews, H, W));
    {
        if (!(regs && vtab_ready)) {
            ProfScope p("pq_vtab");
            if (px) launch_vcol_table(v, nviews, vtab, H, W);
            else STM_LAUNCH(stm_k_vwin_table, dim3(cdiv(G, 4), nT, nviews), dim3(256), 0, stream(), v, vtab, rec, H, W, G, nT, regs ? aggv_table_top() : -1);
            STM_CHECK_LAUNCH();
        }
        if (hregs && !htab_ready) {
            ProfScope p("pq_htab");
            launch_hwin_table(v, nviews, htab, H, W);
        }
    }
    if (from_costs && !fuse_cost) {
        ProfScope p("pq_cost");
        const size_t smem = (size_t)(2 * PC_TX + 2 * (PC_TX + 2 * pad) + 768 + 72) * 4;
        allow_lds_m((const void *)stm_k_pq_cost, smem);
        STM_LAUNCH(stm_k_pq_cost, dim3(cdiv(W, PC_TX), H, nviews), dim3(PC_TX), smem, stream(), v, lut, D, zd, H, W, G, NC, pad);
        STM_CHECK_LAUNCH();
    }
    {
        ProfScope p("pq_h");
        constexpr int NWC = 12;
        const int NGc = 4 * NWC + 2 * HG;
        const size_t smem_c12 = (size_t)4 * NGc * 256 + 16 * NWC * 4 + (size_t)(4 * NGc * 4 + 4 * pad + 768 + 72) * 4;
        const size_t smem_hc = (size_t)4 * NGc * 256 + 16 * NWC * 4 + 8 * NWC + (size_t)(2 * 16 * NWC + 2 * (16 * NWC + 2 * pad)) * 8 + (768 + 72) * 4;
        const int nsegc = cdiv(W, 16 * NWC);
        const size_t smem_hc8 = (size_t)4 * NG * 256 + 16 * NW * 4 + 8 * NW + (size_t)(2 * 16 * NW + 2 * (16 * NW + 2 * pad)) * 8 + (768 + 72) * 4;
        const int hcw = plan.hcw;
#define STM_HC_LAUNCH(NWX, PXS, GRID, SMEM, NSEG, SPL)                                                                                      \
    {                                                                                                                                     \
        allow_lds_m((const void *)stm_k_pq_hc<NWX, PXS>, SMEM);                                                                            \
        STM_LAUNCH((stm_k_pq_hc<NWX, PXS>), GRID, dim3(64 * NWX), SMEM, stream(), v, D, zd, H, W, G, NC, HG, NSEG, SPL, lut, pad, dbgh);    \
    }
        if (plan.hc2_spl) {
            allow_lds_m((const void *)stm_k_pq_hc2, HC2_SMEM);
            STM_LAUNCH(stm_k_pq_hc2, dim3(H * plan.hc2_spl), dim3(768), HC2_SMEM, stream(), v, D, zd, H, W, G, cdiv(W, HC2_TX), plan.hc2_spl, lut, dbgh);
        } else if (hcw == NWC) {
            const dim3 grid(nviews * H * plan.hc_spl);
            if (px) STM_HC_LAUNCH(NWC, true, grid, smem_hc, plan.hc_nseg, plan.hc_spl)
            else STM_HC_LAUNCH(NWC, false, grid, smem_hc, plan.hc_nseg, plan.hc_spl)
        } else if (hcw == NW) {
            const dim3 grid(nviews * H * plan.hc_spl);
            if (px) STM_HC_LAUNCH(NW, true, grid, smem_hc8, plan.hc_nseg, plan.hc_spl)
            else STM_HC_LAUNCH(NW, false, grid, smem_hc8, plan.hc_nseg, plan.hc_spl)
        } else if (fuse_cost && smem_c12 <= 80 * 1024 && (agg_variant() / 1000) % 10 != 1) {
            const int nblkc = ((nsegc * H * nviews + 7) / 8) * 8;
            allow_lds_m((const void *)stm_k_pq_h<NWC, false, true>, smem_c12);
            STM_LAUNCH((stm_k_pq_h<NWC, false, true>), dim3(nblkc), dim3(64 * NWC), smem_c12, stream(), v, D, zd, H, W, G, NC, HG, nsegc, dbgh, lut, pad, nviews);
        } else if (fuse_cost) {
            allow_lds_m((const void *)stm_k_pq_h<NW, false, true>, smem_cost);
            STM_LAUNCH((stm_k_pq_h<NW, false, true>), dim3(nblk), dim3(64 * NW), smem_cost, stream(), v, D, zd, H, W, G, NC, HG, nseg, dbgh, lut, pad, nviews);
        } else if (streaming) {
            allow_lds_m((const void *)stm_k_pq_hs<NW, false>, smem_h);
            STM_LAUNCH((stm_k_pq_hs<NW, false>), dim3(nviews * H * spl), dim3(64 * NW), smem_h, stream(), v, D, zd, H, W, G, NC, HG, nseg, spl, dbgh);
        } else {
            allow_lds_m((const void *)stm_k_pq_h<NW, false, false>, smem_h);
            STM_LAUNCH((stm_k_pq_h<NW, false, false>), dim3(nblk), dim3(64 * NW), smem_h, stream(), v, D, zd, H, W, G, NC, HG, nseg, dbgh, lut, 0, nviews);
        }
#undef STM_HC_LAUNCH
        STM_CHECK_LAUNCH();
    }
    {
        ProfScope p("pq_v12");
        if (px) {
            launch_pq_v12r(v, nviews, vtab, H, W, G);
        } else if (regs) {
            launch_pq_v12q(v, nviews, vtab, rec, H, W, G, NC);
        } else {
            const size_t smem = (size_t)(RQ1 + RQ2) * 1024;
            allow_lds_m((const void *)stm_k_pq_v12t<NTP>, smem);
            STM_LAUNCH(stm_k_pq_v12t<NTP>, dim3(G, NC, nviews), dim3(128 * NTP), smem, stream(), v, vtab, rec, H, W, G, NC, UQ, RQ1, RQ2, LAG, dbgh);
            STM_CHECK_LAUNCH();
        }
    }
    {
        ProfScope p("pq_hw");
        if (hregs) {
            launch_pq_hsr(v, nviews, htab, D, zd, H, W, px);
        } else if (streaming && !wta) {
            allow_lds_m((const void *)stm_k_pq_hs<NW, false>, smem_h);
            STM_LAUNCH((stm_k_pq_hs<NW, false>), dim3(nviews * H * spl), dim3(64 * NW), smem_h, stream(), v, D, zd, H, W, G, NC, HG, nseg, spl, dbgh);
        } else if (streaming) {
            const int splw = NC > 4 ? std::max(spl, cdiv(nseg * 16 * NW, 1920)) : spl;
            const size_t smem_w = smem_h + (NC > 4 ? (size_t)cdiv(nseg, splw) * 16 * NW * 8 : 0);
            allow_lds_m((const void *)stm_k_pq_hs<NW, true>, smem_w);
            STM_LAUNCH((stm_k_pq_hs<NW, true>), dim3(nviews * H * splw), dim3(64 * NW), smem_w, stream(), v, D, zd, H, W, G, NC, HG, nseg, splw, dbgh);
        } else if (!wta) {
            allow_lds_m((const void *)stm_k_pq_h<NW, false, false>, smem_h);
            STM_LAUNCH((stm_k_pq_h<NW, false, false>), dim3(nblk), dim3(64 * NW), smem_h, stream(), v, D, zd, H, W, G, NC, HG, nseg, dbgh, lut, 0, nviews);
        } else {
            allow_lds_m((const void *)stm_k_pq_h<NW, true, false>, smem_h);
            STM_LAUNCH((stm_k_pq_h<NW, true, false>), dim3(nblk), dim3(64 * NW), smem_h, stream(), v, D, zd, H, W, G, NC, HG, nseg, dbgh, lut, 0, nviews);
        }
        STM_CHECK_LAUNCH();
    }
}

size_t aggm_frame_vtab_dwords(int D, int zd, int H, int W, int usd, bool keep_volume, bool v2_read_later, int *rec, int *top, bool *col)
{
    if (usd > 255) usd = 255;
    const bool regs = chain_vregs(usd);
    *col = aggm_frame_px(D, zd, H, W, usd, keep_volume, v2_read_later);
    *rec = !regs ? 0 : *col ? HR_REC : aggv_table_rec();
    *top = regs ? aggv_table_top() : -1;
    if (!regs || (agg_variant() / 1000000000) % 10 == 1) return 0;
    return *col ? aggv_col_table_dwords(2, H, W) : (size_t)2 * ((H + 15) / 16) * ((W + 3) / 4) * *rec;
}
size_t aggm_frame_htab_dwords(int D, int H, int W, int usd, bool keep_volume)
{
    if (usd > 255) usd = 255;
    const bool hregs = chain_hregs(!keep_volume, usd, D);
    return hregs && (agg_variant() / 1000000000) % 10 != 1 ? aggh_table_dwords(2, H, W) : 0;
}
void launch_aggm_frame(const uint32_t *const *pk, const uint32_t *const *cen, const float *lut, float *const *vol_a, float *const *vol_b,
                       const u8 *const *armU, const u8 *const *armD, const u8 *const *armL, const u8 *const *armR, float *const *disp,
                       int D, int zd, int H, int W, int usd, bool keep_volume, uint32_t *htab_ready, uint32_t *vtab_ready, bool v2_read_later)
{
    PQViews v;
    for (int i = 0; i < 2; ++i) {
        v.pk[i] = pk[i]; v.cen[i] = cen[i]; v.a[i] = vol_a[i]; v.b[i] = vol_b[i];
        v.armU[i] = armU[i]; v.armD[i] = armD[i]; v.armL[i] = armL[i]; v.armR[i] = armR[i]; v.disp[i] = disp[i];
    }
    aggm_chain(v, 2, true, !keep_volume, lut, D, zd, H, W, usd, htab_ready, vtab_ready, aggm_frame_px(D, zd, H, W, usd, keep_volume, v2_read_later));
}

static int vtab_rec(int usd)
{
    if (usd > 255) usd = 255;
    const bool regs = chain_vregs(usd);
    return regs ? aggv_table_rec() : 8 + 8 * ((2 * usd + 21) / 4 + 2);
}
size_t aggm_stage_bytes(int D, int H, int W, int usd)
{
    const int G = (W + 3) / 4, nT = (H + 15) / 16;
    return 2 * pq_volume_floats(D, H, W) * sizeof(float) + (size_t)nT * G * vtab_rec(usd) * 4 + 4096;
}
bool launch_aggm_stage(Vol in, Vol out, const u8 *armU, const u8 *armD, const u8 *armL, const u8 *armR, int D, int H, int W, int usd)
{
    const size_t VP = pq_volume_floats(D, H, W);
    float *m = Workspace::get<float>(2 * VP);
    uint32_t *odd = Workspace::get<uint32_t>(64);
    if (failed()) return true;
    STM_CHECK(hipMemsetAsync(odd, 0, 4, stream()));
    PQViews v;
    for (int i = 0; i < 2; ++i) {
        v.pk[i] = nullptr; v.cen[i] = nullptr; v.a[i] = m; v.b[i] = m + VP;
        v.armU[i] = armU; v.armD[i] = armD; v.armL[i] = armL; v.armR[i] = armR; v.disp[i] = nullptr;
    }
    launch_to_pq(in, m, D, H, W, odd);
    uint32_t h_odd = 0;
    STM_CHECK(hipMemcpyAsync(&h_odd, odd, 4, hipMemcpyDeviceToHost, stream()));
    STM_CHECK(hipStreamSynchronize(stream()));
    if (h_odd) return false;
    aggm_chain(v, 1, false, false, nullptr, D, 0, H, W, usd);
    launch_from_pq(m + VP, out, D, H, W);
    return true;
}

}
```

stereo-to-multiview-cuda_amd/csrc/stm_kernels_aggv.hip:

```cpp
#include "stm_hwin.h"

namespace stm {

constexpr int VR_TOP = 36;
constexpr int VR_NQ = 22;

template <int EXP>
__global__ __launch_bounds__(64, 2) void stm_k_pq_v12q(PQViews pv, const uint32_t *__restrict__ wtab, int rec, int H, int G, int NC, int nviews)
{
    int wi = blockIdx.x;
    {
        const int per_xcd = gridDim.x >> 3;
        if (wi < 8 * per_xcd) wi = (wi & 7) * per_xcd + (wi >> 3);
    }
    const int c = wi % NC, sidx = wi / NC;
    if (sidx >= G * nviews) return;
    const int g = sidx % G, view = sidx / G;
    const int l = threadIdx.x;
    const int nT = (H + 15) >> 4;
    const int rsb = G * 256;
    const size_t strip = ((size_t)c * H * G + g) * 64;
    const float *in = (const float *)(view ? pv.b[1] : pv.b[0]) + strip;
    float *out = (float *)(view ? pv.a[1] : pv.a[0]) + strip;
    const uint32_t range = (uint32_t)(H - 1) * (uint32_t)rsb + 256u;
// ... 364 lines not shown
        s_cmp_lt_i32 s24, %[nT]
        s_cselect_b32 s82, s82, 0             ; first-pass tiles past the image: no window rows (their rows are zeros)
        s_sub_i32 s28, s24, 3
        s_mov_b32 s83, s88
        s_cmp_ge_i32 s28, 0
        s_cselect_b32 s84, s89, 0
        .if VR_EXP & 1
        s_mov_b32 s82, 0
        s_mov_b32 s84, 0
        .endif
        ; headers of the tiles of the step after it (tile indices clamped into the table; unused entries are masked above)
        s_sub_u32 s93, %[nT], 1
        s_add_i32 s92, s24, 1
        s_max_i32 s92, s92, 0
        s_min_i32 s92, s92, s93
        s_mul_i32 s92, s92, %[tstep]
        s_load_dwordx2 s[86:87], %[trow], s92
        s_sub_i32 s92, s24, 2
        s_max_i32 s92, s92, 0
        s_min_i32 s92, s92, s93
        s_mul_i32 s92, s92, %[tstep]
        s_load_dwordx2 s[88:89], %[trow], s92
        s_cmp_eq_u32 s82, 0
        s_cbranch_scc1 VR_noissue1_%=_\@
        s_mov_b32 s94, s81
        s_mov_b32 s95, s82
        s_add_u32 s96, s25, 16                ; row 16 u - 36 = row 16 u + 36 - 72, and -72 = 16 (mod 88)
        s_sub_u32 s31, s96, 88
        s_cmp_ge_u32 s96, 88
        s_cselect_b32 s96, s31, s96
        s_movk_i32 s29, 88
        s_mul_i32 s92, s24, %[tstep]
        s_add_u32 s92, s92, 32
        s_add_u32 s98, %[trow_lo], s92
        s_addc_u32 s99, %[trow_hi], 0
        VR_SWEEP_ISSUE
VR_noissue1_%=_\@:
        VR_STORE_ROWS 0
        VR_STORE_ROWS 1
        VR_STORE_ROWS 2
        VR_STORE_ROWS 3
        .endm
VR_loop_%=:
        VR_STEP 88
        s_cmp_ge_i32 s24, s27
        s_cbranch_scc1 VR_done_%=
        VR_STEP 228
        s_cmp_lt_i32 s24, s27
        s_cbranch_scc1 VR_loop_%=
VR_done_%=:
        s_waitcnt vmcnt(0) lgkmcnt(0)         ; the last rows and headers: nothing may be in flight when the wave ends
        .purgem VR_BLOCK
        .purgem VR_PAIR
        .purgem VR_SWEEP_ISSUE
        .purgem VR_SWEEP_RUN
        .purgem VR_ZERO_ACC
        .purgem VR_PUT4
        .purgem VR_LOAD_ROW
        .purgem VR_LOAD_FAST
        .purgem VR_STORE_ROWS
        .purgem VR_STEP
        )ASM"
                 :
                 : [in] "s"(in), [out] "s"(out), [trow] "s"(trow), [trow_lo] "s"((uint32_t)(uintptr_t)trow), [trow_hi] "s"((uint32_t)((uintptr_t)trow >> 32)),
                   [tstep] "s"(tstep), [rsb] "s"(rsb), [H] "s"(H), [nT] "s"(nT), [range] "s"(range), [voff] "v"(voff), [vst] "v"(vst), [exp] "n"(EXP)
                 : "memory", "scc", "vcc",
                   "s16", "s17", "s18", "s19", "s20", "s21", "s22", "s23", "s24", "s25", "s26", "s27", "s29", "s30", "s31", "s36", "s37", "s38", "s39", "s40", "s41", "s42", "s43", "s44", "s45", "s46", "s47", "s48", "s49", "s50", "s51", "s52", "s53", "s54", "s55", "s56", "s57", "s58", "s59", "s60", "s61", "s62", "s63", "s64", "s65", "s66", "s67", "s68", "s69", "s70", "s71", "s72", "s73", "s74", "s75", "s76", "s77", "s78", "s79", "s80", "s81", "s82", "s83", "s84", "s85", "s86", "s87", "s88", "s89", "s90", "s91", "s92", "s93", "s94", "s95", "s96", "s97", "s98", "s99", "s28",
                   "v0", "v1", "v2", "v3", "v4", "v5", "v6", "v7", "v8", "v9", "v10", "v11", "v12", "v13", "v14", "v15", "v16", "v17", "v18", "v19",
                   "v20", "v21", "v22", "v23", "v24", "v25", "v26", "v27", "v28", "v29", "v30", "v31", "v32", "v33", "v34", "v35", "v36", "v37", "v38", "v39",
                   "v40", "v41", "v42", "v43", "v44", "v45", "v46", "v47", "v48", "v49", "v50", "v51", "v52", "v53", "v54", "v55", "v56", "v57", "v58", "v59",
                   "v60", "v61", "v62", "v63", "v64", "v65", "v66", "v67", "v68", "v69", "v70", "v71", "v72", "v73", "v74", "v75", "v76", "v77", "v78", "v79",
                   "v80", "v81", "v82", "v83", "v84", "v85", "v86", "v87", "v88", "v89", "v90", "v91", "v92", "v93", "v94", "v95", "v96", "v97", "v98", "v99",
                   "v100", "v101", "v102", "v103", "v104", "v105", "v106", "v107", "v108", "v109", "v110", "v111", "v112", "v113", "v114", "v115", "v116",
                   "v117", "v118", "v119", "v120", "v121", "v122", "v123", "v124", "v125", "v126", "v127", "v128", "v129", "v130", "v131", "v132", "v133",
                   "v134", "v135", "v136", "v137", "v138", "v139", "v140", "v141", "v142", "v143", "v144", "v145", "v146", "v147", "v148", "v149", "v150",
                   "v151", "v152", "v153", "v154", "v155", "v156", "v157", "v158", "v159", "v160", "v161", "v162", "v163", "v164", "v165", "v166", "v167",
                   "v168", "v169", "v170", "v171", "v172", "v173", "v174", "v175", "v176", "v177", "v178", "v179", "v180", "v181", "v182", "v183", "v184",
                   "v185", "v186", "v187", "v188", "v189", "v190", "v191", "v192", "v193", "v194", "v195", "v196", "v197", "v198", "v199", "v200", "v201",
                   "v202", "v203", "v204", "v205", "v206", "v207", "v208", "v209", "v210", "v211", "v212", "v213", "v214", "v215", "v216", "v217", "v218",
                   "v219", "v220", "v221", "v222", "v223", "v224", "v225", "v226", "v227", "v228", "v229", "v230", "v231", "v232", "v233", "v234", "v235",
                   "v236", "v237", "v238", "v239", "v240", "v241", "v242", "v243", "v244", "v245", "v246", "v247");
}

template <int EXP>
__global__ __launch_bounds__(64, 2) void stm_k_pq_v12r(PQViews pv, const uint32_t *__restrict__ wtab, int H, int G4, int nviews)
{
    const int x = blockIdx.x % G4, view = blockIdx.x / G4;
    if (view >= nviews) return;
    const int l = threadIdx.x;
    const int nT = (H + 15) >> 4;
    const int rsb = G4 * 256;
    const float *in = (const float *)(view ? pv.b[1] : pv.b[0]) + (size_t)x * 64;
    float *out = (float *)(view ? pv.a[1] : pv.a[0]) + (size_t)x * 64;
    const uint32_t range = (uint32_t)(H - 1) * (uint32_t)rsb + 256u;
    const uint32_t *trow = wtab + ((size_t)view * nT * G4 + x) * HR_REC;
    const int tstep = G4 * HR_REC * 4;
    const int voff = 4 * l;
    const int vst = 4 * (l >> 4) * rsb + (l & 15) * 4;
    asm volatile(R"ASM(
        .set VC_EXP, %[exp]
        ; ---------------------------------------------------------------- macros
        ; one block of a sweep: four MFMAs on one quad of ring rows, the A operand (lanes 16 a + m = row a of the quad, tile row m)
        ; shared through CBSZ / ABID.  p = block index, rb = first register of the ring, acur / anxt = the A registers of this / the
        ; next block
        .macro VC_BLOCK p, rb, acur, anxt
        s_set_gpr_idx_idx s30
        v_mfma_f32_16x16x1_4b_f32 v[204:219], v[\acur], v[\rb], v[204:219] cbsz:2 abid:0
        v_cndmask_b32_e64 v[\anxt], 0, 1.0, s[36+2*((\p)+1):37+2*((\p)+1)]
        v_mfma_f32_16x16x1_4b_f32 v[204:219], v[\acur], v[\rb+1], v[204:219] cbsz:2 abid:1
        s_add_u32 s30, s30, 4
        s_cmp_eq_u32 s30, s29
        s_cselect_b32 s30, 0, s30
        v_mfma_f32_16x16x1_4b_f32 v[204:219], v[\acur], v[\rb+2], v[204:219] cbsz:2 abid:2
        v_mfma_f32_16x16x1_4b_f32 v[204:219], v[\acur], v[\rb+3], v[204:219] cbsz:2 abid:3
        .endm
        .macro VC_PAIR b, rb
        VC_BLOCK 2*(\b), \rb, 220, 221
        VC_BLOCK 2*(\b)+1, \rb, 221, 220
        .endm
        ; the loads a sweep starts from.  q0 / n = the tile's header (n in 1 .. 22), s96 = ring index of the range's first row,
        ; s29 = ring size, s[84:85] = the tile's record.  out: s99 = entry block 22 - n, s30 = ring index of the sweep's first row;
        ; in flight: the 24 mask pairs (block p reads pair p + 1 for its successor, the entry block's own comes through M0)
        .macro VC_SWEEP_ISSUE q0, n
        s_sub_u32 s99, 22, \n
        s_lshl_b32 s31, \q0, 2
        s_add_u32 s30, s96, s31
        s_sub_u32 s31, s30, s29
        s_cmp_ge_u32 s30, s29
        s_cselect_b32 s30, s31, s30
        .if (VC_EXP & 4) == 0
        s_load_dwordx16 s[36:51], s[84:85], 0x20
        s_load_dwordx16 s[52:67], s[84:85], 0x60
        s_load_dwordx16 s[68:83], s[84:85], 0xa0
        .endif
        .endm
        ; the sweep: prologue (the entry block's A operand, first MFMA with the constant 0 as accumulator input), computed jump into
        ; the sequence of blocks, epilogue (the accumulators are read by vector instructions next: the last MFMA must have left
        ; the pipe)
        .macro VC_SWEEP_RUN rb
        s_waitcnt lgkmcnt(0)
        s_lshl_b32 m0, s99, 1
        s_nop 0
        s_movrels_b64 s[86:87], s[36:37]      ; the entry block's mask
        v_cndmask_b32_e64 v220, 0, 1.0, s[86:87]
        v_cndmask_b32_e64 v221, 0, 1.0, s[86:87]
        s_set_gpr_idx_on s30, 0x2
        s_mul_i32 s31, s99, 56
        s_getpc_b64 s[84:85]
VC_pc_%=_\@:
        s_add_u32 s31, s31, VC_blk0_%=_\@-VC_pc_%=_\@+12
        s_add_u32 s84, s84, s31
        s_addc_u32 s85, s85, 0
        v_mfma_f32_16x16x1_4b_f32 v[204:219], v220, v[\rb], 0 cbsz:2 abid:0
        s_setpc_b64 s[84:85]
VC_blk0_%=_\@:
        VC_PAIR 0, \rb
        VC_PAIR 1, \rb
        VC_PAIR 2, \rb
        VC_PAIR 3, \rb
        VC_PAIR 4, \rb
        VC_PAIR 5, \rb
        VC_PAIR 6, \rb
        VC_PAIR 7, \rb
        VC_PAIR 8, \rb
        VC_PAIR 9, \rb
        VC_PAIR 10, \rb
VC_end_%=_\@:
        .if (VC_end_%=_\@-VC_blk0_%=_\@) != 22*56
        .error "sweep blocks are not 56 bytes each"
        .endif
        s_set_gpr_idx_off
        s_nop 15
        s_nop 3
        .endm
        .macro VC_ZERO_ACC
        v_mov_b32 v204, 0
        v_mov_b32 v205, 0
        v_mov_b32 v206, 0
        v_mov_b32 v207, 0
        v_mov_b32 v208, 0
        v_mov_b32 v209, 0
        v_mov_b32 v210, 0
        v_mov_b32 v211, 0
// ... 4 lines not shown
        v_mov_b32 v216, 0
        v_mov_b32 v217, 0
        v_mov_b32 v218, 0
        v_mov_b32 v219, 0
        .endm
        ; accumulators (register 4 b + i of lane 16 q + n = [row 4 q + i][chunk b][hypothesis n]) -> row registers (register
        ; 4 q + i of lane 16 b + n): for each i a 4 x 4 transposition of (register b, lane group q)
        .macro VC_TRANSPOSE
        v_permlane32_swap_b32 v204, v212
        v_permlane32_swap_b32 v208, v216
        v_permlane32_swap_b32 v205, v213
        v_permlane32_swap_b32 v209, v217
        v_permlane32_swap_b32 v206, v214
        v_permlane32_swap_b32 v210, v218
        v_permlane32_swap_b32 v207, v215
        v_permlane32_swap_b32 v211, v219
        s_nop 1
        v_permlane16_swap_b32 v204, v208
        v_permlane16_swap_b32 v212, v216
        v_permlane16_swap_b32 v205, v209
        v_permlane16_swap_b32 v213, v217
        v_permlane16_swap_b32 v206, v210
        v_permlane16_swap_b32 v214, v218
        v_permlane16_swap_b32 v207, v211
        v_permlane16_swap_b32 v215, v219
        s_nop 1
        .endm
        ; four registers src.. -> ring registers rb + index.. (relative destination), then index += 4 with wrap at `size` (s31)
        .macro VC_PUT4 rb, src
        v_mov_b32 v[\rb], v[\src]
        v_mov_b32 v[\rb+1], v[\src+1]
        v_mov_b32 v[\rb+2], v[\src+2]
        v_mov_b32 v[\rb+3], v[\src+3]
        s_add_u32 s97, s97, 4
        s_cmp_eq_u32 s97, s31
        s_cselect_b32 s97, 0, s97
        s_set_gpr_idx_idx s97
        .endm
        ; rows are addressed by a scalar offset, which the buffer's range check does not see: a row outside the image goes to an
        ; empty buffer (loads return zeros, stores are dropped), a row of the image passes (its lane offset is below 256)
        .macro VC_LOAD_ROW lb, k
        s_cmp_lt_u32 s86, %[H]
        s_cselect_b32 s18, %[range], 0
        s_mul_i32 s87, s86, %[rsb]
        .if (VC_EXP & 2) == 0
        buffer_load_dword v[\lb+\k], %[voff], s[16:19], s87 offen nt
        .endif
        s_add_u32 s86, s86, 1
        .endm
        .macro VC_LOAD_FAST lb, k
        .if (VC_EXP & 2) == 0
        buffer_load_dword v[\lb+\k], %[voff], s[16:19], s87 offen nt
        .endif
        s_add_u32 s87, s87, %[rsb]
        .endm

        ; ---------------------------------------------------------------- setup
        s_mov_b64 s[16:17], %[in]
        s_and_b32 s17, s17, 0xffff
        s_mov_b32 s18, 0
        s_mov_b32 s19, 0x20000
        s_mov_b64 s[20:21], %[out]
        s_and_b32 s21, s21, 0xffff
        s_mov_b32 s22, 0
        s_mov_b32 s23, 0x20000
        s_mov_b32 s24, -5                     ; u: five steps that only bring rows [0, 52) into ring 1
        s_mov_b32 s25, 44                     ; ring-1 index of row 16 u + 36 = -44
        s_mov_b32 s26, 20                     ; ring-2 index of row 16 u = -80
        s_add_u32 s27, %[nT], 3               ; the second pass runs three tiles behind
        s_mov_b64 s[92:93], 0
        s_mov_b64 s[94:95], 0
        s_mov_b32 s88, 0                      ; the first step has no tiles
        s_mov_b32 s89, 0
        s_mov_b32 s90, 0
        s_mov_b32 s91, 0
        s_sub_i32 s28, s24, 3
        .macro VC_STEP lb
        ; s88 .. s91 = (q0, n) of this step's first-pass tile u and second-pass tile u - 3, s28 = u - 3: set at the end of the step
        ; before, where the masks of this step's first pass were requested too
        ; ------------------------------------------------------------ the rows loaded during the last step -> ring 1
        s_cmp_lt_i32 s24, -3
        s_cbranch_scc1 VC_nocopy_%=_\@
        .if (VC_EXP & 2) == 0
        s_waitcnt vmcnt(48)                   ; the 16 loads of the step before the last (issued since: 16 stores, 16 loads, 16 stores)
        .endif
        .if (VC_EXP & 8) == 0
        s_mov_b32 s97, s25
        s_movk_i32 s31, 88
        s_set_gpr_idx_on s97, 0x8
        VC_PUT4 0, \lb
        VC_PUT4 0, \lb+4
        VC_PUT4 0, \lb+8
        VC_PUT4 0, \lb+12
        s_set_gpr_idx_off
        .endif
VC_nocopy_%=_\@:
        s_cmp_lt_i32 s24, 0
        s_cbranch_scc1 VC_loads_%=_\@
        ; ------------------------------------------------------------ first pass of tile u
        s_cmp_eq_u32 s89, 0
        s_cbranch_scc1 VC_zero1_%=_\@
        VC_SWEEP_RUN 0
        s_branch VC_p1done_%=_\@
VC_zero1_%=_\@:
        VC_ZERO_ACC
VC_p1done_%=_\@:
        ; masks of the second pass (they travel during the transposition and the loads)
        s_cmp_eq_u32 s91, 0
        s_cbranch_scc1 VC_noissue2_%=_\@
        s_add_u32 s96, s26, 16                ; row 16 u - 84, and -84 = 16 (mod 100)
        s_sub_u32 s31, s96, 100
        s_cmp_ge_u32 s96, 100
        s_cselect_b32 s96, s31, s96
        s_movk_i32 s29, 100
        s_mul_i32 s97, s28, %[tstep]
        s_add_u32 s84, %[trow_lo], s97
        s_addc_u32 s85, %[trow_hi], 0
        VC_SWEEP_ISSUE s90, s91
VC_noissue2_%=_\@:
        .if (VC_EXP & 8) == 0
        VC_TRANSPOSE
        ; rows [16 u, 16 u + 16) of the first pass -> ring 2
        s_mov_b32 s97, s26
        s_movk_i32 s31, 100
        s_set_gpr_idx_on s97, 0x8
        VC_PUT4 104, 204
        VC_PUT4 104, 208
        VC_PUT4 104, 212
        VC_PUT4 104, 216
        s_set_gpr_idx_off
        .endif
VC_loads_%=_\@:
        ; ------------------------------------------------------------ rows [16 u + 68, 16 u + 84) -> the landing registers just emptied
        s_lshl_b32 s86, s24, 4
        s_add_i32 s86, s86, 68
        s_add_i32 s87, s86, 15
        s_cmp_lt_u32 s87, %[H]                ; (unsigned: also false for rows above the image)
        s_cbranch_scc0 VC_slowloads_%=_\@
        s_cmp_lt_u32 s86, %[H]
        s_cbranch_scc0 VC_slowloads_%=_\@
        ; all sixteen rows inside the image (every step but the first and the last few): one scalar add per row
        s_mov_b32 s18, %[range]
        s_mul_i32 s87, s86, %[rsb]
        VC_LOAD_FAST \lb, 0
        VC_LOAD_FAST \lb, 1
        VC_LOAD_FAST \lb, 2
        VC_LOAD_FAST \lb, 3
        VC_LOAD_FAST \lb, 4
        VC_LOAD_FAST \lb, 5
        VC_LOAD_FAST \lb, 6
        VC_LOAD_FAST \lb, 7
        VC_LOAD_FAST \lb, 8
        VC_LOAD_FAST \lb, 9
        VC_LOAD_FAST \lb, 10
        VC_LOAD_FAST \lb, 11
        VC_LOAD_FAST \lb, 12
        VC_LOAD_FAST \lb, 13
        VC_LOAD_FAST \lb, 14
        VC_LOAD_FAST \lb, 15
        s_branch VC_loaded_%=_\@
VC_slowloads_%=_\@:
        VC_LOAD_ROW \lb, 0
        VC_LOAD_ROW \lb, 1
        VC_LOAD_ROW \lb, 2
        VC_LOAD_ROW \lb, 3
        VC_LOAD_ROW \lb, 4
        VC_LOAD_ROW \lb, 5
// ... 4 lines not shown
        VC_LOAD_ROW \lb, 10
        VC_LOAD_ROW \lb, 11
        VC_LOAD_ROW \lb, 12
        VC_LOAD_ROW \lb, 13
        VC_LOAD_ROW \lb, 14
        VC_LOAD_ROW \lb, 15
VC_loaded_%=_\@:
        s_cmp_lt_i32 s24, 0
        s_cbranch_scc1 VC_end_of_step_%=_\@
        ; ------------------------------------------------------------ second pass of tile u - 3
        s_cmp_eq_u32 s91, 0
        s_cbranch_scc1 VC_zero2_%=_\@
        VC_SWEEP_RUN 104
        s_branch VC_end_of_step_%=_\@
VC_zero2_%=_\@:
        VC_ZERO_ACC
VC_end_of_step_%=_\@:
        ; the tile's accumulators leave below, behind the next step's bookkeeping.  Always sixteen stores (a step's loads are
        ; counted against them); before tile 0 into an empty buffer
        s_lshl_b32 s86, s28, 4                ; first row of the tile (s86 stays untouched until the stores)
        s_mul_i32 s98, s86, %[rsb]
        ; ------------------------------------------------------------ the next step: ring indices, tiles, masks -- in front of the
        ; stores, so that the masks travel behind them and behind the next step's row moves
        s_add_u32 s25, s25, 16
        s_sub_u32 s31, s25, 88
        s_cmp_ge_u32 s25, 88
        s_cselect_b32 s25, s31, s25
        s_add_u32 s26, s26, 16
        s_sub_u32 s31, s26, 100
        s_cmp_ge_u32 s26, 100
        s_cselect_b32 s26, s31, s26
        s_add_i32 s24, s24, 1
        s_waitcnt lgkmcnt(0)                  ; the headers of its tiles, requested a step ago
        s_mov_b32 s88, s92
        s_cmp_ge_i32 s24, 0
        s_cselect_b32 s89, s93, 0
        s_cmp_lt_i32 s24, %[nT]
        s_cselect_b32 s89, s89, 0             ; first-pass tiles past the image: no window rows (their rows are zeros)
        s_min_u32 s89, s89, 22                ; (the table cannot hold more: the jump must stay inside the sequence)
        s_sub_i32 s28, s24, 3
        s_mov_b32 s90, s94
        s_cmp_ge_i32 s28, 0
        s_cselect_b32 s91, s95, 0
        s_min_u32 s91, s91, 22
        .if VC_EXP & 1
        s_mov_b32 s89, 0
        s_mov_b32 s91, 0
        .endif
        ; headers of the tiles of the step after it (tile indices clamped into the table; unused entries are masked above)
        s_sub_u32 s96, %[nT], 1
        s_add_i32 s97, s24, 1
        s_max_i32 s97, s97, 0
        s_min_i32 s97, s97, s96
        s_mul_i32 s97, s97, %[tstep]
        s_load_dwordx2 s[92:93], %[trow], s97
        s_sub_i32 s97, s24, 2
        s_max_i32 s97, s97, 0
        s_min_i32 s97, s97, s96
        s_mul_i32 s97, s97, %[tstep]
        s_load_dwordx2 s[94:95], %[trow], s97
        s_cmp_eq_u32 s89, 0
        s_cbranch_scc1 VC_noissue1_%=_\@
        s_add_u32 s96, s25, 16                ; row 16 u - 36 = row 16 u + 36 - 72, and -72 = 16 (mod 88)
        s_sub_u32 s31, s96, 88
        s_cmp_ge_u32 s96, 88
        s_cselect_b32 s96, s31, s96
        s_movk_i32 s29, 88
        s_mul_i32 s97, s24, %[tstep]
        s_add_u32 s84, %[trow_lo], s97
        s_addc_u32 s85, %[trow_hi], 0
        VC_SWEEP_ISSUE s88, s89
VC_noissue1_%=_\@:
        ; straight from the accumulators: register 4 b + i of lane 16 q + n = row 4 q + i, hypothesis 16 b + n.  The whole row
        ; offset is in the vector register, so the range check sees it (rows past the image are dropped); before tile 0: empty buffer
        s_cmp_ge_i32 s86, 0
        s_cselect_b32 s22, %[range], 0
        v_add_u32 v224, s98, %[vst]
        s_add_u32 s98, s98, %[rsb]
        v_add_u32 v225, s98, %[vst]
        s_add_u32 s98, s98, %[rsb]
        v_add_u32 v226, s98, %[vst]
        s_add_u32 s98, s98, %[rsb]
        v_add_u32 v227, s98, %[vst]
        .if (VC_EXP & 2) == 0
        buffer_store_dword v204, v224, s[20:23], 0 offen nt
        buffer_store_dword v208, v224, s[20:23], 0 offen offset:64 nt
        buffer_store_dword v212, v224, s[20:23], 0 offen offset:128 nt
        buffer_store_dword v216, v224, s[20:23], 0 offen offset:192 nt
        buffer_store_dword v205, v225, s[20:23], 0 offen nt
        buffer_store_dword v209, v225, s[20:23], 0 offen offset:64 nt
        buffer_store_dword v213, v225, s[20:23], 0 offen offset:128 nt
        buffer_store_dword v217, v225, s[20:23], 0 offen offset:192 nt
        buffer_store_dword v206, v226, s[20:23], 0 offen nt
        buffer_store_dword v210, v226, s[20:23], 0 offen offset:64 nt
        buffer_store_dword v214, v226, s[20:23], 0 offen offset:128 nt
        buffer_store_dword v218, v226, s[20:23], 0 offen offset:192 nt
        buffer_store_dword v207, v227, s[20:23], 0 offen nt
        buffer_store_dword v211, v227, s[20:23], 0 offen offset:64 nt
        buffer_store_dword v215, v227, s[20:23], 0 offen offset:128 nt
        buffer_store_dword v219, v227, s[20:23], 0 offen offset:192 nt
        .endif
        .endm
VC_loop_%=:
        VC_STEP 88
        s_cmp_ge_i32 s24, s27
        s_cbranch_scc1 VC_done_%=
        VC_STEP 228
        s_cmp_lt_i32 s24, s27
        s_cbranch_scc1 VC_loop_%=
VC_done_%=:
        s_waitcnt vmcnt(0) lgkmcnt(0)         ; the last rows, masks and headers: nothing may be in flight when the wave ends
        .purgem VC_BLOCK
        .purgem VC_PAIR
        .purgem VC_SWEEP_ISSUE
        .purgem VC_SWEEP_RUN
        .purgem VC_ZERO_ACC
        .purgem VC_TRANSPOSE
        .purgem VC_PUT4
        .purgem VC_LOAD_ROW
        .purgem VC_LOAD_FAST
        .purgem VC_STEP
        )ASM"
                 :
                 : [in] "s"(in), [out] "s"(out), [trow] "s"(trow), [trow_lo] "s"((uint32_t)(uintptr_t)trow), [trow_hi] "s"((uint32_t)((uintptr_t)trow >> 32)),
                   [tstep] "s"(tstep), [rsb] "s"(rsb), [H] "s"(H), [nT] "s"(nT), [range] "s"(range), [voff] "v"(voff), [vst] "v"(vst), [exp] "n"(EXP)
                 : "memory", "scc", "vcc",
                   "s16", "s17", "s18", "s19", "s20", "s21", "s22", "s23", "s24", "s25", "s26", "s27", "s28", "s29", "s30", "s31", "s36", "s37", "s38", "s39", "s40", "s41", "s42", "s43", "s44", "s45", "s46", "s47", "s48", "s49", "s50", "s51", "s52", "s53", "s54", "s55", "s56", "s57", "s58", "s59", "s60", "s61", "s62", "s63", "s64", "s65", "s66", "s67", "s68", "s69", "s70", "s71", "s72", "s73", "s74", "s75", "s76", "s77", "s78", "s79", "s80", "s81", "s82", "s83", "s84", "s85", "s86", "s87", "s88", "s89", "s90", "s91", "s92", "s93", "s94", "s95", "s96", "s97", "s98", "s99",
                   "v0", "v1", "v2", "v3", "v4", "v5", "v6", "v7", "v8", "v9", "v10", "v11", "v12", "v13", "v14", "v15", "v16", "v17", "v18", "v19",
                   "v20", "v21", "v22", "v23", "v24", "v25", "v26", "v27", "v28", "v29", "v30", "v31", "v32", "v33", "v34", "v35", "v36", "v37", "v38", "v39",
                   "v40", "v41", "v42", "v43", "v44", "v45", "v46", "v47", "v48", "v49", "v50", "v51", "v52", "v53", "v54", "v55", "v56", "v57", "v58", "v59",
                   "v60", "v61", "v62", "v63", "v64", "v65", "v66", "v67", "v68", "v69", "v70", "v71", "v72", "v73", "v74", "v75", "v76", "v77", "v78", "v79",
                   "v80", "v81", "v82", "v83", "v84", "v85", "v86", "v87", "v88", "v89", "v90", "v91", "v92", "v93", "v94", "v95", "v96", "v97", "v98", "v99",
                   "v100", "v101", "v102", "v103", "v104", "v105", "v106", "v107", "v108", "v109", "v110", "v111", "v112", "v113", "v114", "v115", "v116",
                   "v117", "v118", "v119", "v120", "v121", "v122", "v123", "v124", "v125", "v126", "v127", "v128", "v129", "v130", "v131", "v132", "v133",
                   "v134", "v135", "v136", "v137", "v138", "v139", "v140", "v141", "v142", "v143", "v144", "v145", "v146", "v147", "v148", "v149", "v150",
                   "v151", "v152", "v153", "v154", "v155", "v156", "v157", "v158", "v159", "v160", "v161", "v162", "v163", "v164", "v165", "v166", "v167",
                   "v168", "v169", "v170", "v171", "v172", "v173", "v174", "v175", "v176", "v177", "v178", "v179", "v180", "v181", "v182", "v183", "v184",
                   "v185", "v186", "v187", "v188", "v189", "v190", "v191", "v192", "v193", "v194", "v195", "v196", "v197", "v198", "v199", "v200", "v201",
                   "v202", "v203", "v204", "v205", "v206", "v207", "v208", "v209", "v210", "v211", "v212", "v213", "v214", "v215", "v216", "v217", "v218",
                   "v219", "v220", "v221", "v224", "v225", "v226", "v227", "v228", "v229", "v230", "v231", "v232", "v233", "v234", "v235",
                   "v236", "v237", "v238", "v239", "v240", "v241", "v242", "v243");
}

__global__ __launch_bounds__(256) void stm_k_vcol_table(PQViews v, uint32_t *__restrict__ tab, int H, int W, int G, int nT)
{
    __shared__ uint32_t ev_all[4][4 * 96];
    const int l = threadIdx.x & 63, wv = threadIdx.x >> 6, g = blockIdx.x * 4 + wv, u = blockIdx.y, view = blockIdx.z;
    if (g >= G) return;
    const u8 *__restrict__ armU = view ? v.armU[1] : v.armU[0], *__restrict__ armD = view ? v.armD[1] : v.armD[0];
    const int c = l >> 4, m = l & 15, y = u * 16 + m, x = 4 * g + c;
    int s0 = 0, nn = 0;
    if (y < H && x < W) {
        const int aU = armU[(size_t)y * W + x], aD = armD[(size_t)y * W + x];
        s0 = y - aU;
        nn = aU + aD;
    }
    vcol_build(tab + (size_t)(view * nT + u) * (4 * G) * HR_REC, ev_all[wv], u, 4 * g, s0, nn);
}

bool aggv_supports(int usd) { return usd >= 1 && usd <= VR_TOP; }
int aggv_table_top() { return VR_TOP; }
int aggv_table_rec() { return 8 + 8 * (VR_NQ + 2); }

void launch_pq_v12q(PQViews &v, int nviews, const uint32_t *tab, int rec, int H, int W, int G, int NC)
{
    (void)W;
    const dim3 grid(G * nviews * NC);
#ifdef STM_TIMING
    switch (timing_knobs()) {
    case 1: STM_LAUNCH(stm_k_pq_v12q<1>, grid, dim3(64), 0, stream(), v, tab, rec, H, G, NC, nviews); break;
    case 2: STM_LAUNCH(stm_k_pq_v12q<2>, grid, dim3(64), 0, stream(), v, tab, rec, H, G, NC, nviews); break;
    case 3: STM_LAUNCH(stm_k_pq_v12q<3>, grid, dim3(64), 0, stream(), v, tab, rec, H, G, NC, nviews); break;
    case 4: STM_LAUNCH(stm_k_pq_v12q<4>, grid, dim3(64), 0, stream(), v, tab, rec, H, G, NC, nviews); break;
    case 6: STM_LAUNCH(stm_k_pq_v12q<6>, grid, dim3(64), 0, stream(), v, tab, rec, H, G, NC, nviews); break;
    case 8: STM_LAUNCH(stm_k_pq_v12q<8>, grid, dim3(64), 0, stream(), v, tab, rec, H, G, NC, nviews); break;
    case 9: STM_LAUNCH(stm_k_pq_v12q<9>, grid, dim3(64), 0, stream(), v, tab, rec, H, G, NC, nviews); break;
    default: STM_LAUNCH(stm_k_pq_v12q<0>, grid, dim3(64), 0, stream(), v, tab, rec, H, G, NC, nviews); break;
    }
#else
    STM_LAUNCH(stm_k_pq_v12q<0>, grid, dim3(64), 0, stream(), v, tab, rec, H, G, NC, nviews);
#endif
    STM_CHECK_LAUNCH();
}


size_t aggv_col_table_dwords(int nviews, int H, int W) { return (size_t)nviews * cdiv(H, 16) * (4 * cdiv(W, 4)) * HR_REC + 64; }

void launch_vcol_table(PQViews &v, int nviews, uint32_t *tab, int H, int W)
{
    const int G = cdiv(W, 4), nT = cdiv(H, 16);
    STM_LAUNCH(stm_k_vcol_table, dim3(cdiv(G, 4), nT, nviews), dim3(256), 0, stream(), v, tab, H, W, G, nT);
    STM_CHECK_LAUNCH();
}

void launch_pq_v12r(PQViews &v, int nviews, const uint32_t *tab, int H, int W, int G)
{
    (void)W;
    const int G4 = 4 * G;
    const dim3 grid(G4 * nviews);
#define STM_V12R_LAUNCH(E) STM_LAUNCH(stm_k_pq_v12r<E>, grid, dim3(64), 0, stream(), v, tab, H, G4, nviews)
#ifdef STM_TIMING
    switch (timing_knobs()) {
    case 1: STM_V12R_LAUNCH(1); break;
    case 2: STM_V12R_LAUNCH(2); break;
    case 3: STM_V12R_LAUNCH(3); break;
    case 4: STM_V12R_LAUNCH(4); break;
    case 8: STM_V12R_LAUNCH(8); break;
    default: STM_V12R_LAUNCH(0); break;
    }
#else
    STM_V12R_LAUNCH(0);
#endif
#undef STM_V12R_LAUNCH
    STM_CHECK_LAUNCH();
}

}
```

stereo-to-multiview-cuda_amd/device_api.py:

```python
import ctypes as C

import torch

from ._lib import f32p, f32pp, lib


def _use_current_stream():
    lib().stm_set_stream(C.c_void_p(torch.cuda.current_stream().cuda_stream))


def _p(t):
    return C.c_void_p(t.data_ptr())


STAGE_SUBPIXEL = 0x200
STAGE_INTERP = 0x400
STAGE_LINEAR_WARP = 0x800
STAGE_GUIDED_UP = 0x1000
STAGE_TEMPORAL = 0x2000
TEMPORAL_DEFAULTS = (0.5, 24, 1.5)


class FrameParams:

    def __init__(self, num_disp=64, zero_disp=32, num_views=8, angle=18.43, ad_coeff=10.0, census_coeff=30.0,
                 ucd=6.0, lcd=20.0, usd=34, lsd=17, thresh_s=20, thresh_h=0.4, out_rows=None, out_cols=None):
        self.num_disp, self.zero_disp, self.num_views, self.angle = num_disp, zero_disp, num_views, angle
        self.ad_coeff, self.census_coeff = ad_coeff, census_coeff
        self.ucd, self.lcd, self.usd, self.lsd = ucd, lcd, usd, lsd
        self.thresh_s, self.thresh_h = thresh_s, thresh_h
        self.out_rows, self.out_cols = out_rows, out_cols


AGG_MATRIX_PIPE, AGG_PX, AGG_VREGS, AGG_HREGS, AGG_SPLIT = 1, 2, 4, 8, 1 << 16


def agg_path(num_disp, zero_disp, num_rows, num_cols, usd, stages=3):
    return int(lib().stm_agg_path(int(num_disp), int(zero_disp), int(num_rows), int(num_cols), int(usd), int(stages)))


def agg_path_waves(path):
    return (int(path) >> 8) & 0xff


def first_pass_path(num_disp, zero_disp, num_rows, num_cols, usd, stages=3):
    return int(lib().stm_first_pass_path(int(num_disp), int(zero_disp), int(num_rows), int(num_cols), int(usd), int(stages)))


IRV_PRUNE, IRV_RUNS, IRV_CHAIN = 1, 2, 4


def irv_path(num_rows, num_cols, usd, iterations=5, device_flavour=True, with_dcc=False):
    return int(lib().stm_irv_path(int(num_rows), int(num_cols), int(usd), int(iterations), int(bool(device_flavour)), int(bool(with_dcc))))


def irv_path_tile_sh(path):
    return (int(path) >> 8) & 0xf


def irv_path_chunk(path):
    return (int(path) >> 16) & 0x1f


def set_irv_chunk(entries=0):
    if int(lib().stm_set_irv_chunk(int(entries))) != 0:
        raise ValueError("stm_set_irv_chunk(%d) refused: %s" % (entries, lib().stm_last_error().decode()))


def set_lens(mode, pitch=0.0, slope=0.0, centre=0.0):
    if int(lib().stm_set_lens(int(mode), float(pitch), float(slope), float(centre))) != 0:
        raise ValueError("stm_set_lens(%d, %g, %g, %g) refused: %s" % (mode, pitch, slope, centre, lib().stm_last_error().decode()))


def set_layout(layout=0, tiles_x=1, tiles_y=1, order=0, filter=0):
    if int(lib().stm_set_layout(int(layout), int(tiles_x), int(tiles_y), int(order), int(filter))) != 0:
        raise ValueError("stm_set_layout(%d, %d, %d, %d, %d) refused: %s"
                         % (layout, tiles_x, tiles_y, order, filter, lib().stm_last_error().decode()))


def get_layout():
    out = (C.c_int * 5)()
    lib().stm_get_layout(out)
    return tuple(int(v) for v in out)


def set_output(format=0, matrix=0, pitch=0, uv_row=0):
    if int(lib().stm_set_output(int(format), int(matrix), int(pitch), int(uv_row))) != 0:
        raise ValueError("stm_set_output(%d, %d, %d, %d) refused: %s" % (format, matrix, pitch, uv_row, lib().stm_last_error().decode()))


def get_output():
    out = (C.c_int * 4)()
    lib().stm_get_output(out)
    return tuple(int(v) for v in out)


_overlay_keepalive = {}


def _check_overlay(overlay):
    assert overlay.is_cuda and overlay.dtype == torch.uint8 and overlay.is_contiguous()
    assert overlay.dim() == 3 and overlay.shape[2] == 4, "an overlay is uint8 [rows][cols][4]: B, G, R, A, premultiplied"


def set_overlay(d_overlay, x0=0, y0=0, disparity=0.0):
    import threading
    if d_overlay is None:
        lib().stm_set_overlay(0, None, 0, 0, 0, 0, 0.0)
        _overlay_keepalive.pop(threading.get_ident(), None)
        return
    _check_overlay(d_overlay)
    if int(lib().stm_set_overlay(1, _p(d_overlay), d_overlay.shape[0], d_overlay.shape[1], int(x0), int(y0), float(disparity))) != 0:
        raise ValueError("stm_set_overlay(%d x %d at (%d, %d), disparity %g) refused: %s"
                         % (d_overlay.shape[0], d_overlay.shape[1], x0, y0, disparity, lib().stm_last_error().decode()))
    _overlay_keepalive[threading.get_ident()] = d_overlay


def get_overlay():
    out = (C.c_int * 5)()
    disp = C.c_float(0.0)
    lib().stm_get_overlay(out, C.cast(C.byref(disp), f32p))
    return tuple(int(v) for v in out) + (float(disp.value),)


def d_mux_overlay(frame, overlay, x0, y0, disparity, num_views, angle=18.43, lens=None, layout=None):
    assert frame.is_cuda and frame.dtype == torch.uint8 and frame.dim() == 3 and frame.is_contiguous()
    _check_overlay(overlay)
    ln = tuple(lens) if lens is not None else (0, 0.0, 0.0, 0.0)
    lo = tuple(layout)[:4] if layout is not None else (0, 1, 1, 0)
# ... 538 lines not shown
```

Baseline: 670.3 frames/s.

## Interleave disparity order in px aggregation buffer for dwordx4 stores

Adds a second disparity ordering for the per-pixel intermediate buffer used by the matrix-pipe aggregation chain. Within each 16-disparity group, disparities are interleaved so each lane holds four consecutive values. The horizontal-cost kernels and the vertical v12r kernel can then write 16-byte vector stores instead of four scalar dword stores, and the horizontal WTA/scan kernel reads in the new order. It is enabled by default when the px path is used, with an agg_variant digit to fall back. The cost is extra register moves and a layout that every producer and consumer must agree on.

After: 684.1 frames/s (median of 6 runs). +2.1%, better.

```diff
diff --git a/include/stm_hip.h b/include/stm_hip.h
--- a/include/stm_hip.h
+++ b/include/stm_hip.h
@@ -20,6 +20,7 @@
 void        stm_set_agg_variant(int v);
 int         stm_agg_path(int num_disp, int zero_disp, int num_rows, int num_cols, int usd, int stages);
 int         stm_first_pass_path(int num_disp, int zero_disp, int num_rows, int num_cols, int usd, int stages);
+int         stm_px_order(int num_disp, int zero_disp, int num_rows, int num_cols, int usd, int stages);
 void        stm_set_irv_paper_ratio(int on);
 int         stm_set_irv_chunk(int entries);
 int         stm_irv_path(int num_rows, int num_cols, int usd, int iterations, int device_flavour, int with_dcc);
diff --git a/stereo-to-multiview-cuda_amd/_lib.py b/stereo-to-multiview-cuda_amd/_lib.py
--- a/stereo-to-multiview-cuda_amd/_lib.py
+++ b/stereo-to-multiview-cuda_amd/_lib.py
@@ -27,6 +27,7 @@
     "stm_set_agg_variant": ([i], None),
     "stm_agg_path": ([i, i, i, i, i, i], i),
     "stm_first_pass_path": ([i, i, i, i, i, i], i),
+    "stm_px_order": ([i, i, i, i, i, i], i),
     "stm_set_irv_paper_ratio": ([i], None),
     "stm_set_irv_chunk": ([i], i),
     "stm_irv_path": ([i, i, i, i, i, i], i),
diff --git a/stereo-to-multiview-cuda_amd/csrc/stm_api.hip b/stereo-to-multiview-cuda_amd/csrc/stm_api.hip
--- a/stereo-to-multiview-cuda_amd/csrc/stm_api.hip
+++ b/stereo-to-multiview-cuda_amd/csrc/stm_api.hip
@@ -157,6 +157,11 @@
 {
     if (D < 1 || H < 1 || W < 1 || !agg_on_matrix_pipe(usd, H, W)) return 0;
     return aggm_frame_hc2_parts(D, zd, H, W, usd, stages_hslo(stages), stages_subpix(stages));
+}
+int frame_px_order(int D, int zd, int H, int W, int usd, int stages)
+{
+    if (D < 1 || H < 1 || W < 1 || !agg_on_matrix_pipe(usd, H, W)) return -1;
+    return aggm_frame_px_order(D, zd, H, W, usd, stages_hslo(stages), stages_subpix(stages));
 }
 void core_agg(Vol cost, Vol scratch, const Arms &a, int D, int H, int W, int usd)
 {
@@ -2013,6 +2018,10 @@
 {
     return frame_first_pass_path(num_disp, zero_disp, num_rows, num_cols, usd, stages);
 }
+int stm_px_order(int num_disp, int zero_disp, int num_rows, int num_cols, int usd, int stages)
+{
+    return frame_px_order(num_disp, zero_disp, num_rows, num_cols, usd, stages);
+}
 
 void stm_d_adcensus_stm(unsigned char *d_img_sbs, float *d_disp_l, float *d_disp_r, unsigned char *d_interlaced,
                         int num_rows, int num_cols_sbs, int num_cols, int num_rows_out, int num_cols_out, int elem_sz,
diff --git a/stereo-to-multiview-cuda_amd/csrc/stm_common.h b/stereo-to-multiview-cuda_amd/csrc/stm_common.h
--- a/stereo-to-multiview-cuda_amd/csrc/stm_common.h
+++ b/stereo-to-multiview-cuda_amd/csrc/stm_common.h
@@ -350,6 +350,7 @@
 size_t aggm_frame_htab_dwords(int D, int H, int W, int usd, bool keep_volume);
 size_t aggm_frame_vtab_dwords(int D, int zd, int H, int W, int usd, bool keep_volume, bool v2_read_later, int *rec, int *top, bool *col);
 bool aggm_frame_px(int D, int zd, int H, int W, int usd, bool keep_volume, bool v2_read_later);
+int aggm_frame_px_order(int D, int zd, int H, int W, int usd, bool keep_volume, bool v2_read_later);
 int aggm_frame_path(int D, int zd, int H, int W, int usd, bool keep_volume, bool v2_read_later);
 int aggm_frame_hc2_parts(int D, int zd, int H, int W, int usd, bool keep_volume, bool v2_read_later);
 bool launch_aggm_stage(Vol in, Vol out, const u8 *armU, const u8 *armD, const u8 *armL, const u8 *armR, int D, int H, int W, int usd);
@@ -357,12 +358,12 @@
 bool aggh_supports(int usd, int D);
 size_t aggh_table_dwords(int nviews, int H, int W);
 void launch_hwin_table(PQViews &v, int nviews, uint32_t *tab, int H, int W);
-void launch_pq_hsr(PQViews &v, int nviews, const uint32_t *tab, int D, int zd, int H, int W, bool px = false);
+void launch_pq_hsr(PQViews &v, int nviews, const uint32_t *tab, int D, int zd, int H, int W, bool px = false, int ord = 0);
 bool aggv_supports(int usd);
 int aggv_table_top();
 int aggv_table_rec();
 void launch_pq_v12q(PQViews &v, int nviews, const uint32_t *tab, int rec, int H, int W, int G, int NC);
-void launch_pq_v12r(PQViews &v, int nviews, const uint32_t *tab, int H, int W, int G);
+void launch_pq_v12r(PQViews &v, int nviews, const uint32_t *tab, int H, int W, int G, bool x4 = false);
 void launch_vcol_table(PQViews &v, int nviews, uint32_t *tab, int H, int W);
 size_t aggv_col_table_dwords(int nviews, int H, int W);
 void launch_to_pq(Vol in, float *pq, int D, int H, int W, uint32_t *odd = nullptr);
diff --git a/stereo-to-multiview-cuda_amd/csrc/stm_kernels_aggh.hip b/stereo-to-multiview-cuda_amd/csrc/stm_kernels_aggh.hip
--- a/stereo-to-multiview-cuda_amd/csrc/stm_kernels_aggh.hip
+++ b/stereo-to-multiview-cuda_amd/csrc/stm_kernels_aggh.hip
@@ -19,7 +19,7 @@
 
 template <int EXP, bool PX>
 __global__ __launch_bounds__(64, 3) void stm_k_pq_hsr(PQViews pv, const uint32_t *__restrict__ htab, int D, int zd, int H, int W, int G, int NC, int nTx,
-                                                      int parts, int nviews)
+                                                      int parts, int nviews, int ord)
 {
     const int part = blockIdx.x % parts, rest = blockIdx.x / parts, y = rest % H, view = rest / H;
     if (view >= nviews) return;
@@ -32,11 +32,13 @@
     const uint32_t cstride = (uint32_t)H * (uint32_t)G * 256u;
     const uint32_t nrec = (uint32_t)NC * cstride;
     const int vload = PX ? 4 * l : (l >> 4) * (int)cstride + (l & 15) * 16;
-    const int vn = l & 15;
+    const int hstep = PX && ord ? 1 : 16;
+    const int vn = PX && ord ? 4 * (l & 15) : l & 15;
+    const int hs2 = 2 * hstep, hs3 = 3 * hstep;
     const int vst = (l & 15) == 0 ? (l >> 4) * 16 : 0x7ffffff0;
     float vbig[4];
 #pragma unroll
-    for (int b = 0; b < 4; ++b) vbig[b] = (16 * b + (l & 15)) >= D ? 3.402823466e+38f : 0.0f;
+    for (int b = 0; b < 4; ++b) vbig[b] = (vn + b * hstep) >= D ? 3.402823466e+38f : 0.0f;
     const int yG = y * G, Gm1 = G - 1, W4 = W * 4;
     const float zdf = (float)zd;
     asm volatile(R"ASM(
@@ -281,7 +283,7 @@
         v_max_f32 v134, v134, %[vb3]
         v_max_f32 v135, v135, %[vb3]
 HR_nofix_%=_\@:
-        ; per lane: the lowest of its four chunks, the lower chunk on ties; v[138:141] = that hypothesis (d = 16 b + n)
+        ; per lane: the lowest of its four chunks, the lower chunk (= the lower d) on ties; v[138:141] = that hypothesis (v151 .. v153)
         HR_WTA_CHUNK 1, 151
         HR_WTA_CHUNK 2, 152
         HR_WTA_CHUNK 3, 153
@@ -338,9 +340,9 @@
         s_mov_b32 s31, 0
         HR_NEXT_MASKS
         v_mov_b32 v150, 0x7fffffff
-        v_add_u32 v151, 16, %[vn]
-        v_add_u32 v152, 32, %[vn]
-        v_add_u32 v153, 48, %[vn]
+        v_add_u32 v151, %[hs1], %[vn]
+        v_add_u32 v152, %[hs2], %[vn]
+        v_add_u32 v153, %[hs3], %[vn]
         v_or_b32 v146, %[vb0], %[vb1]
         v_or3_b32 v146, v146, %[vb2], %[vb3]
         v_cmp_ne_u32 vcc, 0, v146
@@ -411,7 +413,7 @@
         )ASM"
                  :
                  : [exp] "n"(EXP), [px] "n"(PX ? 1 : 0), [in] "s"(in), [disp] "s"(disp_row), [hrec_lo] "s"((uint32_t)(uintptr_t)hrec), [hrec_hi] "s"((uint32_t)((uintptr_t)hrec >> 32)),
-                   [yG] "s"(yG), [Gm1] "s"(Gm1), [nrec] "s"(nrec), [W4] "s"(W4), [t0] "s"(t0), [t1] "s"(t1), [zdf] "s"(zdf),
+                   [yG] "s"(yG), [Gm1] "s"(Gm1), [nrec] "s"(nrec), [W4] "s"(W4), [t0] "s"(t0), [t1] "s"(t1), [zdf] "s"(zdf), [hs1] "s"(hstep), [hs2] "s"(hs2), [hs3] "s"(hs3),
                    [vload] "v"(vload), [vn] "v"(vn), [vst] "v"(vst), [vb0] "v"(vbig[0]),
                    [vb1] "v"(vbig[1]), [vb2] "v"(vbig[2]), [vb3] "v"(vbig[3])
                  : "memory", "scc", "vcc",
@@ -441,7 +443,7 @@
     STM_CHECK_LAUNCH();
 }
 
-void launch_pq_hsr(PQViews &v, int nviews, const uint32_t *tab, int D, int zd, int H, int W, bool px)
+void launch_pq_hsr(PQViews &v, int nviews, const uint32_t *tab, int D, int zd, int H, int W, bool px, int ord)
 {
     const int G = (W + 3) / 4, NC = (D + 15) / 16, nTx = cdiv(W, 16);
     int parts = (nTx + 5) / 10;
@@ -449,8 +451,8 @@
     const dim3 grid(nviews * H * parts);
 #define STM_HSR_LAUNCH(E, GRID)                                                                                                       \
     {                                                                                                                                 \
-        if (px) STM_LAUNCH((stm_k_pq_hsr<E, true>), GRID, dim3(64), 0, stream(), v, tab, D, zd, H, W, G, NC, nTx, parts, nviews);      \
-        else STM_LAUNCH((stm_k_pq_hsr<E, false>), GRID, dim3(64), 0, stream(), v, tab, D, zd, H, W, G, NC, nTx, parts, nviews);        \
+        if (px) STM_LAUNCH((stm_k_pq_hsr<E, true>), GRID, dim3(64), 0, stream(), v, tab, D, zd, H, W, G, NC, nTx, parts, nviews, ord); \
+        else STM_LAUNCH((stm_k_pq_hsr<E, false>), GRID, dim3(64), 0, stream(), v, tab, D, zd, H, W, G, NC, nTx, parts, nviews, 0);     \
     }
 #ifdef STM_TIMING
     if (const char *e = getenv("STM_HSR_PARTS")) parts = atoi(e);
diff --git a/stereo-to-multiview-cuda_amd/csrc/stm_kernels_aggm.hip b/stereo-to-multiview-cuda_amd/csrc/stm_kernels_aggm.hip
--- a/stereo-to-multiview-cuda_amd/csrc/stm_kernels_aggm.hip
+++ b/stereo-to-multiview-cuda_amd/csrc/stm_kernels_aggm.hip
@@ -476,7 +476,7 @@
 #undef STM_HS_SN
 }
 
-template <int NW, bool PX>
+template <int NW, bool PX, int ORD>
 __global__ __launch_bounds__(64 * NW, (2 * NW) / 4) void stm_k_pq_hc(PQViews v, int D, int zd, int H, int W, int G, int NC, int HG, int nseg,
                                                                      int spl, const float *__restrict__ lut_g, int pad, int dbg)
 {
@@ -664,12 +664,18 @@
                     const f4 o = {acc[4 * cl], acc[4 * cl + 1], acc[4 * cl + 2], acc[4 * cl + 3]};
                     if (!STM_DBG(dbg, 4)) STM_BSTORE(rout[cl], (X0 >> 2) * 256 + l * 16, o);
                 }
-            } else {
+            } else if (ORD == 0) {
 #pragma unroll
                 for (int k = 0; k < 16; ++k)
                     if (!STM_DBG(dbg, 4))
                         __builtin_amdgcn_raw_buffer_store_b32(__builtin_bit_cast(uint32_t, (float)acc[k]), rpx,
                                                               (X0 + 4 * lb + (k & 3)) * 256 + (16 * (k >> 2) + dd) * 4, 0, 2);
+            } else {
+#pragma unroll
+                for (int i = 0; i < 4; ++i) {
+                    const f4 o = {acc[i], acc[4 + i], acc[8 + i], acc[12 + i]};
+                    if (!STM_DBG(dbg, 4)) STM_BSTORE(rpx, (X0 + 4 * lb + i) * 256 + 16 * dd, o);
+                }
             }
         }
         if (more) STM_HC_COSTS((sq + 1) & 1, 4 * NW * (sq + 1) + NG - 4 * NW)
@@ -697,6 +703,7 @@
 constexpr int HC2_TX = 96, HC2_SR = HC2_TX + 64, HC2_HALO = 40, HC2_RING = 256, HC2_FRONT = HC2_TX + HC2_HALO;
 typedef const float __attribute__((address_space(3))) *hc2_lds_cf;
 constexpr size_t HC2_SMEM =(size_t)(HC2_RING + 3) * 256 + 2 * HC2_TX * 4 + 12 * 8 + (size_t)(2 * HC2_TX + 2 * HC2_SR) * 8 + (768 + 72) * 4;
+template <int ORD>
 __global__ __launch_bounds__(768, 6) void stm_k_pq_hc2(PQViews v, int D, int zd, int H, int W, int G, int nseg, int spl,
                                                        const float *__restrict__ lut_g, int dbg)
 {
@@ -853,11 +860,19 @@
 #pragma unroll
                 for (int i = 0; i < 16; ++i) acc[i] = 0.f;
             }
-#pragma unroll
-            for (int k = 0; k < 16; ++k)
-                if (!STM_DBG(dbg, 4))
-                    __builtin_amdgcn_raw_buffer_store_b32(__builtin_bit_cast(uint32_t, (float)acc[k]), rpx,
-                                                          (X0 + 4 * lb + (k & 3)) * 256 + (16 * (k >> 2) + dd) * 4, 0, 2);
+            if (ORD == 0) {
+#pragma unroll
+                for (int k = 0; k < 16; ++k)
+                    if (!STM_DBG(dbg, 4))
+                        __builtin_amdgcn_raw_buffer_store_b32(__builtin_bit_cast(uint32_t, (float)acc[k]), rpx,
+                                                              (X0 + 4 * lb + (k & 3)) * 256 + (16 * (k >> 2) + dd) * 4, 0, 2);
+            } else {
+#pragma unroll
+                for (int i = 0; i < 4; ++i) {
+                    const f4 o = {acc[i], acc[4 + i], acc[8 + i], acc[12 + i]};
+                    if (!STM_DBG(dbg, 4)) STM_BSTORE(rpx, (X0 + 4 * lb + i) * 256 + 16 * dd, o);
+                }
+            }
         }
         if (more) STM_HC2_COSTS((sq + 1) & 1)
         __syncthreads();
@@ -1168,6 +1183,12 @@
     (void)W;
     return !v2_read_later && chain_px(true, !keep_volume, D, zd, usd);
 }
+static int px_order() { return (agg_variant() / 1000000000) % 10 == 2 ? 0 : 2; }
+int aggm_frame_px_order(int D, int zd, int H, int W, int usd, bool keep_volume, bool v2_read_later)
+{
+    if (usd > 255) usd = 255;
+    return aggm_frame_px(D, zd, H, W, usd, keep_volume, v2_read_later) ? px_order() : -1;
+}
 
 constexpr int HC2_SLOTS = 2 * 256;
 static int hc2_parts(bool px, int D, int zd, int H, int W, int usd)
@@ -1227,6 +1248,7 @@
     const bool fuse_cost = from_costs && (agg_variant() / 1000000) % 10 != 1;
     const int spl = row_split(nseg);
     const ChainPlan plan = chain_plan(from_costs, wta, D, zd, H, W, usd, px && nviews == 2);
+    const int ord = px ? px_order() : 0;
     const bool streaming = NG / 4 >= NW && (agg_variant() / 10) % 10 != 1 && (NC <= 4 || (agg_variant() / 10) % 10 != 2);
     constexpr int NTP = 3, TS = 16 * NTP;
     const int UQ = (usd + 3) & ~3, nT = (H + 15) / 16;
@@ -1265,22 +1287,29 @@
         const int nsegc = cdiv(W, 16 * NWC);
         const size_t smem_hc8 = (size_t)4 * NG * 256 + 16 * NW * 4 + 8 * NW + (size_t)(2 * 16 * NW + 2 * (16 * NW + 2 * pad)) * 8 + (768 + 72) * 4;
         const int hcw = plan.hcw;
-#define STM_HC_LAUNCH(NWX, PXS, GRID, SMEM, NSEG, SPL)                                                                                      \
-    {                                                                                                                                     \
-        allow_lds_m((const void *)stm_k_pq_hc<NWX, PXS>, SMEM);                                                                            \
-        STM_LAUNCH((stm_k_pq_hc<NWX, PXS>), GRID, dim3(64 * NWX), SMEM, stream(), v, D, zd, H, W, G, NC, HG, NSEG, SPL, lut, pad, dbgh);    \
+#define STM_HC_LAUNCH(NWX, PXS, ORD, GRID, SMEM, NSEG, SPL)                                                                                     \
+    {                                                                                                                                          \
+        allow_lds_m((const void *)stm_k_pq_hc<NWX, PXS, ORD>, SMEM);                                                                            \
+        STM_LAUNCH((stm_k_pq_hc<NWX, PXS, ORD>), GRID, dim3(64 * NWX), SMEM, stream(), v, D, zd, H, W, G, NC, HG, NSEG, SPL, lut, pad, dbgh);    \
+    }
+#define STM_HC2_LAUNCH(ORD)                                                                                                                          \
+    {                                                                                                                                               \
+        allow_lds_m((const void *)stm_k_pq_hc2<ORD>, HC2_SMEM);                                                                                      \
+        STM_LAUNCH(stm_k_pq_hc2<ORD>, dim3(H * plan.hc2_spl), dim3(768), HC2_SMEM, stream(), v, D, zd, H, W, G, cdiv(W, HC2_TX), plan.hc2_spl, lut, dbgh); \
     }
         if (plan.hc2_spl) {
-            allow_lds_m((const void *)stm_k_pq_hc2, HC2_SMEM);
-            STM_LAUNCH(stm_k_pq_hc2, dim3(H * plan.hc2_spl), dim3(768), HC2_SMEM, stream(), v, D, zd, H, W, G, cdiv(W, HC2_TX), plan.hc2_spl, lut, dbgh);
+            if (ord) STM_HC2_LAUNCH(1)
+            else STM_HC2_LAUNCH(0)
         } else if (hcw == NWC) {
             const dim3 grid(nviews * H * plan.hc_spl);
-            if (px) STM_HC_LAUNCH(NWC, true, grid, smem_hc, plan.hc_nseg, plan.hc_spl)
-            else STM_HC_LAUNCH(NWC, false, grid, smem_hc, plan.hc_nseg, plan.hc_spl)
+            if (px && ord) STM_HC_LAUNCH(NWC, true, 1, grid, smem_hc, plan.hc_nseg, plan.hc_spl)
+            else if (px) STM_HC_LAUNCH(NWC, true, 0, grid, smem_hc, plan.hc_nseg, plan.hc_spl)
+            else STM_HC_LAUNCH(NWC, false, 0, grid, smem_hc, plan.hc_nseg, plan.hc_spl)
         } else if (hcw == NW) {
             const dim3 grid(nviews * H * plan.hc_spl);
-            if (px) STM_HC_LAUNCH(NW, true, grid, smem_hc8, plan.hc_nseg, plan.hc_spl)
-            else STM_HC_LAUNCH(NW, false, grid, smem_hc8, plan.hc_nseg, plan.hc_spl)
+            if (px && ord) STM_HC_LAUNCH(NW, true, 1, grid, smem_hc8, plan.hc_nseg, plan.hc_spl)
+            else if (px) STM_HC_LAUNCH(NW, true, 0, grid, smem_hc8, plan.hc_nseg, plan.hc_spl)
+            else STM_HC_LAUNCH(NW, false, 0, grid, smem_hc8, plan.hc_nseg, plan.hc_spl)
         } else if (fuse_cost && smem_c12 <= 80 * 1024 && (agg_variant() / 1000) % 10 != 1) {
             const int nblkc = ((nsegc * H * nviews + 7) / 8) * 8;
             allow_lds_m((const void *)stm_k_pq_h<NWC, false, true>, smem_c12);
@@ -1296,12 +1325,13 @@
             STM_LAUNCH((stm_k_pq_h<NW, false, false>), dim3(nblk), dim3(64 * NW), smem_h, stream(), v, D, zd, H, W, G, NC, HG, nseg, dbgh, lut, 0, nviews);
         }
 #undef STM_HC_LAUNCH
+#undef STM_HC2_LAUNCH
         STM_CHECK_LAUNCH();
     }
     {
         ProfScope p("pq_v12");
         if (px) {
-            launch_pq_v12r(v, nviews, vtab, H, W, G);
+            launch_pq_v12r(v, nviews, vtab, H, W, G, ord == 2);
         } else if (regs) {
             launch_pq_v12q(v, nviews, vtab, rec, H, W, G, NC);
         } else {
@@ -1314,7 +1344,7 @@
     {
         ProfScope p("pq_hw");
         if (hregs) {
-            launch_pq_hsr(v, nviews, htab, D, zd, H, W, px);
+            launch_pq_hsr(v, nviews, htab, D, zd, H, W, px, ord);
         } else if (streaming && !wta) {
             allow_lds_m((const void *)stm_k_pq_hs<NW, false>, smem_h);
             STM_LAUNCH((stm_k_pq_hs<NW, false>), dim3(nviews * H * spl), dim3(64 * NW), smem_h, stream(), v, D, zd, H, W, G, NC, HG, nseg, spl, dbgh);
diff --git a/stereo-to-multiview-cuda_amd/csrc/stm_kernels_aggv.hip b/stereo-to-multiview-cuda_amd/csrc/stm_kernels_aggv.hip
--- a/stereo-to-multiview-cuda_amd/csrc/stm_kernels_aggv.hip
+++ b/stereo-to-multiview-cuda_amd/csrc/stm_kernels_aggv.hip
@@ -470,7 +470,7 @@
                    "v236", "v237", "v238", "v239", "v240", "v241", "v242", "v243", "v244", "v245", "v246", "v247");
 }
 
-template <int EXP>
+template <int EXP, bool X4>
 __global__ __launch_bounds__(64, 2) void stm_k_pq_v12r(PQViews pv, const uint32_t *__restrict__ wtab, int H, int G4, int nviews)
 {
     const int x = blockIdx.x % G4, view = blockIdx.x / G4;
@@ -484,9 +484,10 @@
     const uint32_t *trow = wtab + ((size_t)view * nT * G4 + x) * HR_REC;
     const int tstep = G4 * HR_REC * 4;
     const int voff = 4 * l;
-    const int vst = 4 * (l >> 4) * rsb + (l & 15) * 4;
+    const int vst = 4 * (l >> 4) * rsb + (l & 15) * (X4 ? 16 : 4);
     asm volatile(R"ASM(
         .set VC_EXP, %[exp]
+        .set VC_X4, %[x4]
         ; ---------------------------------------------------------------- macros
         ; one block of a sweep: four MFMAs on one quad of ring rows, the A operand (lanes 16 a + m = row a of the quad, tile row m)
         ; shared through CBSZ / ABID.  p = block index, rb = first register of the ring, acur / anxt = the A registers of this / the
@@ -657,7 +658,11 @@
         s_cmp_lt_i32 s24, -3
         s_cbranch_scc1 VC_nocopy_%=_\@
         .if (VC_EXP & 2) == 0
+        .if VC_X4
+        s_waitcnt vmcnt(24)                   ; the 16 loads of the step before the last (issued since: 4 stores, 16 loads, 4 stores)
+        .else
         s_waitcnt vmcnt(48)                   ; the 16 loads of the step before the last (issued since: 16 stores, 16 loads, 16 stores)
+        .endif
         .endif
         .if (VC_EXP & 8) == 0
         s_mov_b32 s97, s25
@@ -828,7 +833,37 @@
         v_add_u32 v226, s98, %[vst]
         s_add_u32 s98, s98, %[rsb]
         v_add_u32 v227, s98, %[vst]
+        .if VC_X4
+        ; the tuples of rows i = 0 .. 3, two register sets in turn (a set is rewritten five instructions after its store)
+        v_mov_b32 v244, v204
+        v_mov_b32 v245, v208
+        v_mov_b32 v246, v212
+        v_mov_b32 v247, v216
         .if (VC_EXP & 2) == 0
+        buffer_store_dwordx4 v[244:247], v224, s[20:23], 0 offen nt
+        .endif
+        v_mov_b32 v248, v205
+        v_mov_b32 v249, v209
+        v_mov_b32 v250, v213
+        v_mov_b32 v251, v217
+        .if (VC_EXP & 2) == 0
+        buffer_store_dwordx4 v[248:251], v225, s[20:23], 0 offen nt
+        .endif
+        v_mov_b32 v244, v206
+        v_mov_b32 v245, v210
+        v_mov_b32 v246, v214
+        v_mov_b32 v247, v218
+        .if (VC_EXP & 2) == 0
+        buffer_store_dwordx4 v[244:247], v226, s[20:23], 0 offen nt
+        .endif
+        v_mov_b32 v248, v207
+        v_mov_b32 v249, v211
+        v_mov_b32 v250, v215
+        v_mov_b32 v251, v219
+        .if (VC_EXP & 2) == 0
+        buffer_store_dwordx4 v[248:251], v227, s[20:23], 0 offen nt
+        .endif
+        .elseif (VC_EXP & 2) == 0
         buffer_store_dword v204, v224, s[20:23], 0 offen nt
         buffer_store_dword v208, v224, s[20:23], 0 offen offset:64 nt
         buffer_store_dword v212, v224, s[20:23], 0 offen offset:128 nt
@@ -869,7 +904,7 @@
         )ASM"
                  :
                  : [in] "s"(in), [out] "s"(out), [trow] "s"(trow), [trow_lo] "s"((uint32_t)(uintptr_t)trow), [trow_hi] "s"((uint32_t)((uintptr_t)trow >> 32)),
-                   [tstep] "s"(tstep), [rsb] "s"(rsb), [H] "s"(H), [nT] "s"(nT), [range] "s"(range), [voff] "v"(voff), [vst] "v"(vst), [exp] "n"(EXP)
+                   [tstep] "s"(tstep), [rsb] "s"(rsb), [H] "s"(H), [nT] "s"(nT), [range] "s"(range), [voff] "v"(voff), [vst] "v"(vst), [exp] "n"(EXP), [x4] "n"(X4 ? 1 : 0)
                  : "memory", "scc", "vcc",
                    "s16", "s17", "s18", "s19", "s20", "s21", "s22", "s23", "s24", "s25", "s26", "s27", "s28", "s29", "s30", "s31", "s36", "s37", "s38", "s39", "s40", "s41", "s42", "s43", "s44", "s45", "s46", "s47", "s48", "s49", "s50", "s51", "s52", "s53", "s54", "s55", "s56", "s57", "s58", "s59", "s60", "s61", "s62", "s63", "s64", "s65", "s66", "s67", "s68", "s69", "s70", "s71", "s72", "s73", "s74", "s75", "s76", "s77", "s78", "s79", "s80", "s81", "s82", "s83", "s84", "s85", "s86", "s87", "s88", "s89", "s90", "s91", "s92", "s93", "s94", "s95", "s96", "s97", "s98", "s99",
                    "v0", "v1", "v2", "v3", "v4", "v5", "v6", "v7", "v8", "v9", "v10", "v11", "v12", "v13", "v14", "v15", "v16", "v17", "v18", "v19",
@@ -885,7 +920,7 @@
                    "v185", "v186", "v187", "v188", "v189", "v190", "v191", "v192", "v193", "v194", "v195", "v196", "v197", "v198", "v199", "v200", "v201",
                    "v202", "v203", "v204", "v205", "v206", "v207", "v208", "v209", "v210", "v211", "v212", "v213", "v214", "v215", "v216", "v217", "v218",
                    "v219", "v220", "v221", "v224", "v225", "v226", "v227", "v228", "v229", "v230", "v231", "v232", "v233", "v234", "v235",
-                   "v236", "v237", "v238", "v239", "v240", "v241", "v242", "v243");
+                   "v236", "v237", "v238", "v239", "v240", "v241", "v242", "v243", "v244", "v245", "v246", "v247", "v248", "v249", "v250", "v251");
 }
 
 __global__ __launch_bounds__(256) void stm_k_vcol_table(PQViews v, uint32_t *__restrict__ tab, int H, int W, int G, int nT)
@@ -939,12 +974,16 @@
     STM_CHECK_LAUNCH();
 }
 
-void launch_pq_v12r(PQViews &v, int nviews, const uint32_t *tab, int H, int W, int G)
+void launch_pq_v12r(PQViews &v, int nviews, const uint32_t *tab, int H, int W, int G, bool x4)
 {
     (void)W;
     const int G4 = 4 * G;
     const dim3 grid(G4 * nviews);
-#define STM_V12R_LAUNCH(E) STM_LAUNCH(stm_k_pq_v12r<E>, grid, dim3(64), 0, stream(), v, tab, H, G4, nviews)
+#define STM_V12R_LAUNCH(E)                                                                                  \
+    {                                                                                                       \
+        if (x4) STM_LAUNCH((stm_k_pq_v12r<E, true>), grid, dim3(64), 0, stream(), v, tab, H, G4, nviews);   \
+        else STM_LAUNCH((stm_k_pq_v12r<E, false>), grid, dim3(64), 0, stream(), v, tab, H, G4, nviews);     \
+    }
 #ifdef STM_TIMING
     switch (timing_knobs()) {
     case 1: STM_V12R_LAUNCH(1); break;
diff --git a/stereo-to-multiview-cuda_amd/device_api.py b/stereo-to-multiview-cuda_amd/device_api.py
--- a/stereo-to-multiview-cuda_amd/device_api.py
+++ b/stereo-to-multiview-cuda_amd/device_api.py
@@ -45,6 +45,10 @@
 
 def first_pass_path(num_disp, zero_disp, num_rows, num_cols, usd, stages=3):
     return int(lib().stm_first_pass_path(int(num_disp), int(zero_disp), int(num_rows), int(num_cols), int(usd), int(stages)))
+
+
+def px_order(num_disp, zero_disp, num_rows, num_cols, usd, stages=3):
+    return int(lib().stm_px_order(int(num_disp), int(zero_disp), int(num_rows), int(num_cols), int(usd), int(stages)))
 
 
 IRV_PRUNE, IRV_RUNS, IRV_CHAIN = 1, 2, 4
```
